# yuw444/fastF

Measured on AMD Instinct MI355X. Metric: BAM records/sec -> deduped UMI matrix; achieved HBM GB/s vs roofline, higher is better.
Workload: dtype u64

## Files before the change

fastf_amd/_lib.py:

```python
import ctypes as C
import os
import subprocess

HERE = os.path.dirname(os.path.abspath(__file__))
ROOT = os.path.dirname(HERE)
_LIB = os.environ.get("FASTF_LIB_OVERRIDE") or os.path.join(HERE, "lib", "libfastf_amd.so")
_CLI = os.path.join(HERE, "bin", "fastF")


class FastfError(RuntimeError):
    pass


def lib_path():
    return _LIB


def cli_path():
    return _CLI


def build(force=False):
    args = ["make", "-s", "-C", os.path.join(HERE, "csrc")]
    if force:
# ... 80 lines not shown
    "fastf_cap_summary_row", "fastf_cap_thresholds", "fastf_cap_realised", "fastf_dev_cell_hits", "fastf_dev_cell_decisions",
]


def _one_hip_runtime():
    import importlib.util
    import sys
    if "torch" in sys.modules or os.environ.get("FASTF_SYSTEM_HIP") == "1":
        return
    try:
        spec = importlib.util.find_spec("torch")
    except (ImportError, ValueError):
        spec = None
    if spec is None or not spec.origin:
        return
    rt = os.path.join(os.path.dirname(spec.origin), "lib", "libamdhip64.so")
    if os.path.exists(rt):
        C.CDLL(rt, mode=C.RTLD_GLOBAL)


def hip_runtimes_loaded():
    with open("/proc/self/maps") as f:
        return sorted({ln.split()[-1] for ln in f if "libamdhip64" in ln})


def lib():
    global _lib
    if _lib is not None:
        return _lib
    if not os.path.exists(_LIB):
        raise FastfError("%s is missing: run `python -c 'import __graft_entry__ as g; g.build()'` "
                         "(there is no Python/CPU fallback for the engine)" % _LIB)
    _one_hip_runtime()
    L = C.CDLL(_LIB, mode=C.RTLD_GLOBAL)
    vp, u64, u32, sz = C.c_void_p, C.c_uint64, C.c_uint32, C.c_size_t
    L.fastf_last_error.restype = C.c_char_p
    L.fastf_version.restype = C.c_char_p
    L.fastf_kernel_names.restype = C.c_char_p
    L.fastf_dev_probe_capacity.argtypes = [vp, u64, C.POINTER(u64)]
    L.fastf_engine_push_pinned.argtypes = [vp, vp]
    L.fastf_engine_wait_input.argtypes = [vp]
    L.fastf_pinned_alloc.argtypes = [sz]
    L.fastf_pinned_alloc.restype = vp
    L.fastf_pinned_free.argtypes = [vp]
    L.fastf_pinned_register.argtypes = [vp, sz]
    L.fastf_pinned_unregister.argtypes = [vp]
    L.fastf_mt_seed.argtypes = [C.POINTER(MT), u32]
    L.fastf_mt_next.argtypes = [C.POINTER(MT)]
    L.fastf_mt_next.restype = u32
    L.fastf_mt_fill.argtypes = [C.POINTER(MT), vp, sz]
    L.fastf_mt_skip.argtypes = [C.POINTER(MT), u64]
    L.fastf_draw_threshold.argtypes = [C.c_float]
    L.fastf_draw_threshold.restype = u64
    L.fastf_sample_cells.argtypes = [sz, C.c_float, C.c_uint, vp, C.POINTER(sz), C.POINTER(u64)]
    L.fastf_pack_umi.argtypes = [C.c_char_p, sz, C.POINTER(u32)]
    L.fastf_pack_umi.restype = u32
    L.fastf_keydict_create.restype = vp
    L.fastf_keydict_destroy.argtypes = [vp]
    L.fastf_keydict_add.argtypes = [vp, C.c_char_p, sz]
    L.fastf_keydict_add.restype = u64
    L.fastf_keydict_pack.argtypes = [vp, C.c_char_p, sz]
    L.fastf_keydict_pack.restype = u64
    L.fastf_keydict_pack_many.argtypes = [vp, vp, sz, sz, vp, vp]
    L.fastf_keydict_pack_many.restype = None
    L.fastf_engine_create.argtypes = [C.POINTER(EngineConfig), C.POINTER(vp)]
    L.fastf_engine_destroy.argtypes = [vp]
    L.fastf_engine_destroy.restype = None
    L.fastf_engine_push.argtypes = [vp, C.POINTER(Batch)]
    L.fastf_engine_push_draws.argtypes = [vp, C.POINTER(Batch), vp, sz]
    L.fastf_engine_finish.argtypes = [vp, C.POINTER(Coo), C.POINTER(u64 * 3)]
    L.fastf_engine_lend_rows.argtypes = [vp, vp, sz]
    L.fastf_engine_umi_rows.argtypes = [vp, C.POINTER(UmiRows)]
    L.fastf_engine_reset.argtypes = [vp]
    L.fastf_engine_device_records.argtypes = [vp, C.POINTER(u64), u32]
    L.fastf_engine_reseed.argtypes = [vp, u32, u64]
    L.fastf_engine_key_bits.argtypes = [vp, C.POINTER(u32), C.POINTER(u32), C.POINTER(u32), C.POINTER(u32)]
    L.fastf_engine_set_timing.argtypes = [vp, C.c_int]
    L.fastf_engine_get_timing.argtypes = [vp, C.c_int, C.POINTER(C.c_double), C.POINTER(u64)]
    L.fastf_dev_count_hits.argtypes = [vp, vp, u64, vp, vp]
    L.fastf_dev_count_hits_blocked.argtypes = [vp, vp, u64, vp, vp, vp]
    L.fastf_dev_block_bytes.argtypes = [vp, u64, C.POINTER(u64)]
    L.fastf_dev_block_records.argtypes = [vp, vp, vp, vp, u64, vp, vp]
    L.fastf_dev_set_regions.argtypes = [vp, vp, u32, u64, vp, vp]
    if hasattr(L, "fastf_dev_draw_bits") or not os.environ.get("FASTF_LIB_OVERRIDE"):
        L.fastf_dev_draw_bits.argtypes = [vp, vp, u64, vp, vp]
    if hasattr(L, "fastf_dev_mt_decisions"):
        L.fastf_dev_mt_decisions.argtypes = [vp, u32, u64, u64, vp, vp]
    L.fastf_dev_probe_pack.argtypes = [vp, vp, vp, vp, vp, u64, vp, u64, vp, vp, u64, vp, vp, u32, vp]
    if hasattr(L, "fastf_dev_probe_pack_wide"):
        L.fastf_dev_probe_pack_wide.argtypes = [vp, vp, vp, vp, vp, vp, u64, vp, u64, vp, vp, vp, u64, vp, vp, u32, vp]
        L.fastf_dev_adopt_wide.argtypes = [vp, vp, vp, u64, vp]
        L.fastf_engine_is_wide.argtypes = [vp]
    L.fastf_dev_sort.argtypes = [vp, vp, vp, vp, u64, u32, u32, C.POINTER(C.c_int), vp]
    L.fastf_dev_reduce.argtypes = [vp, vp, vp, u64, vp, vp, vp, vp, u32, vp]
    L.fastf_dev_rows_gather.argtypes = [vp, vp, vp, vp, vp, vp]
    L.fastf_engine_skip_bits.argtypes = [vp, C.POINTER(u32)]
    L.fastf_engine_sort_passes.argtypes = [vp, u32, C.POINTER(u32)]
    L.fastf_engine_table_modes.argtypes = [vp, C.POINTER(C.c_int), C.POINTER(C.c_int)]
    L.fastf_dev_umi_rows.argtypes = [vp, vp, vp, u64, vp, vp, vp, vp]
    L.fastf_dev_reserve.argtypes = [vp, u64, u64]
    L.fastf_dev_error_bits.argtypes = [vp, C.POINTER(u64)]
    L.fastf_dev_clear_error_bits.argtypes = [vp, u64, vp]
    L.fastf_lists_load_mem.argtypes = [C.c_char_p, sz, C.c_char_p, sz, C.c_float, C.c_uint, C.POINTER(ListsStruct)]
    L.fastf_lists_load.argtypes = [C.c_char_p, C.c_char_p, C.c_float, C.c_uint, C.POINTER(ListsStruct)]
    L.fastf_lists_free.argtypes = [C.POINTER(ListsStruct)]
    L.fastf_lists_free.restype = None
    L.fastf_bam_open.argtypes = [C.c_char_p, C.c_int]
    L.fastf_bam_open.restype = vp
    L.fastf_bam_read_batch.argtypes = [vp, vp, vp, vp, vp, vp, vp, sz]
    L.fastf_bam_read_batch.restype = C.c_long
    L.fastf_bam_close.argtypes = [vp]
    L.fastf_bam_close.restype = None
    L.fastf_bam_stats.argtypes = [vp, C.POINTER(C.c_uint64), C.POINTER(C.c_uint64), C.POINTER(C.c_uint64)]
    L.fastf_bam_stats.restype = None
    L.fastf_format_matrix.argtypes = [C.c_char_p, C.c_float, C.c_float, C.POINTER(u64 * 3), sz, sz,
                                      C.POINTER(Coo), C.POINTER(vp), C.POINTER(sz)]
    L.fastf_format_umi_rows.argtypes = [C.POINTER(UmiRows), C.POINTER(vp), C.POINTER(sz)]
    L.fastf_keydict_intern.argtypes = [vp, C.c_char_p, sz]
    L.fastf_keydict_intern.restype = u64
    L.fastf_keydict_decode.argtypes = [vp, u64, C.c_char_p, sz]
    L.fastf_keydict_decode.restype = C.c_long
    L.fastf_taghist_create.argtypes = [C.c_int, C.POINTER(vp)]
    L.fastf_taghist_destroy.argtypes = [vp]
    L.fastf_taghist_destroy.restype = None
    L.fastf_taghist_push.argtypes = [vp, vp, vp, sz]
    L.fastf_taghist_finish.argtypes = [vp, C.POINTER(TagHistResult)]
    L.fastf_crb_text.argtypes = [C.c_char_p, C.POINTER(vp), C.POINTER(sz), C.POINTER(u64)]
    L.fastf_extract_text.argtypes = [C.c_char_p, C.c_char_p, C.c_int, C.POINTER(vp), C.POINTER(sz), C.POINTER(u64), C.POINTER(u64)]
    L.fastf_freq_text.argtypes = [C.c_char_p, sz, sz, C.POINTER(vp), C.POINTER(sz), C.POINTER(u64)]
    L.fastf_filter.argtypes = [C.c_char_p, C.c_char_p, C.c_char_p, C.c_char_p, C.c_char_p, C.c_uint32, C.c_uint32, C.c_float,
                               C.c_int, C.POINTER(u64), C.POINTER(u64)]
    L.fastf_filter_draws.argtypes = [C.c_uint32, u64, u64, vp]
    L.fastf_filter_draws_host.argtypes = [C.c_uint32, u64, u64, vp]
    L.fastf_filter_rand_at.argtypes = [C.c_uint32, u64]
    L.fastf_filter_rand_at.restype = C.c_uint32
    L.fastf_filter_draw_passes.argtypes = [C.c_uint32, C.c_float]
    L.fastf_taghist_reserve_device.argtypes = [vp, sz]
    L.fastf_taghist_reserve_device.restype = vp
    L.fastf_taghist_stream.argtypes = [vp]
    L.fastf_taghist_stream.restype = vp
    L.fastf_taghist_push_device.argtypes = [vp, vp, sz]
    L.fastf_bam_read_tags.argtypes = [vp, vp, C.c_char_p, C.c_char_p, C.c_int, vp, vp, sz, C.POINTER(u64)]
    L.fastf_bam_read_tags.restype = C.c_long
    L.read_bam.argtypes = [C.c_char_p]
    L.read_bam.restype = vp
    L.print_CB_node.argtypes = [vp, vp]
    L.print_CB_node.restype = None
    L.free_CB_node.argtypes = [vp]
    L.free_CB_node.restype = None
    L.extract_bam.argtypes = [C.c_char_p, C.c_char_p, C.c_int]
    L.extract_bam.restype = None
    fp = C.POINTER(C.c_float)
    L.fastf_sweep.argtypes = [C.c_char_p, C.c_char_p, C.c_char_p, C.c_char_p, fp, u32, fp, u32, u32, u32]
    L.fastf_sweep_parse_rates.argtypes = [C.c_char_p, C.c_int, fp, u32, C.POINTER(u32)]
    L.fastf_sweep_check_grid.argtypes = [fp, u32, fp, u32]
    L.fastf_sweep_point_dir.argtypes = [C.c_float, C.c_float, C.c_char_p, sz]
    L.fastf_sweep_header.restype = C.c_char_p
    L.fastf_sweep_cells_from_coo.argtypes = [C.POINTER(Coo), u32, vp, vp, C.POINTER(u64)]
    L.fastf_sweep_summary_row.argtypes = [C.c_float, C.c_float, u32, C.POINTER(u64 * 3), u64, u64, vp, vp, u32, C.c_char_p, sz]
    L.fastf_dev_mt_decisions_multi.argtypes = [vp, u32, u64, u64, vp, u32, vp, u64, vp]
    L.fastf_dev_cell_summary.argtypes = [vp, vp, vp, vp, u32, vp, vp, vp]
    L.fastf_cap.argtypes = [C.c_char_p, C.c_char_p, C.c_char_p, C.c_char_p, fp, u32, vp, u32, u32, u32]
    L.fastf_cap_parse_caps.argtypes = [C.c_char_p, vp, u32, C.POINTER(u32)]
    L.fastf_cap_check_grid.argtypes = [fp, u32, vp, u32]
    L.fastf_cap_point_dir.argtypes = [C.c_float, u64, C.c_char_p, sz]
    L.fastf_cap_header.restype = C.c_char_p
# ... 15 lines not shown
```

fastf_amd/csrc/umi_engine.hip:

```cpp
#include "umi_kernels.hpp"
#include "sweep_kernels.hpp"
#include "cap_kernels.hpp"

#include <algorithm>
#include <cstdarg>
#include <cstdio>
#include <cstdlib>
#include <cstring>
#include <mutex>
#include <new>
#include <stdexcept>
#include <chrono>
#include <string>
#include <thread>
#include <vector>

extern "C" {
#include "fastf_amd.h"
#include "host_io.h"
#include "mt_jump.h"
}

using namespace fastf;

// ... 123 lines not shown
static int copy_h2d_on(void* d_dst, const void* h_src, size_t bytes, hipStream_t s) {
    std::lock_guard<std::mutex> lk(g_bounce.mu);
    if (g_bounce.ready()) return 1;
    for (size_t o = 0; o < bytes; o += HostBounce::BYTES) {
        const size_t n = std::min(bytes - o, HostBounce::BYTES);
        memcpy(g_bounce.p, (const char*)h_src + o, n);
        HIP_OK(hipMemcpyAsync((char*)d_dst + o, g_bounce.p, n, hipMemcpyHostToDevice, s));
        HIP_OK(hipStreamSynchronize(s));
    }
    return 0;
}

struct KernelTimer {
    std::vector<std::pair<hipEvent_t, hipEvent_t>> ev;
    size_t used = 0;
};

struct fastf_multi;
struct fastf_engine {
    fastf_multi* multi = nullptr;
    int device = 0;
    hipStream_t s_compute = nullptr, s_copy = nullptr, s_mt = nullptr;
    hipEvent_t ev_mt = nullptr;
    KeyLayout L{};
    u32 cell_bits = 0, feat_bits = 0, n_cells = 0, n_features = 0;
    u64 threshold = 0;
    u32 n_shards = 1, shard_rank = 0;
    DevBuf tab_cells, tab_feats;
    Table cells{}, feats{};
    DevBuf img_cells, img_genes;
    DevBuf d_cell_filter; MissFilter cell_filter{nullptr, 0};
    CellLds lds_cells{}; GeneLds lds_genes{};
    bool cell16 = false;
    bool use_lds_cells = false, use_lds_genes = false; u32 genes_blocks_per_cu = 1, cells_blocks_per_cu = 1;
    fastf_mt_t mt{};
    u32 mt_seed0 = 0; u64 mt_skip0 = 0;
    u64 mt_hits = 0;
    u64 mt_abs0 = 0;
    bool mt_live = false;
    DevBuf d_ring; u64 ring_len = 0;
    u32 ring_carry = 0;
    DevBuf d_dbits;
    DevBuf d_mtwords;
    bool mtwords_kept = false; u32 mtwords_seed = 0; u64 mtwords_skip = 0, mtwords_n = 0;
    bool cap_lds_attr = false;
    DevBuf d_mt; bool mt_on_device = false;
    u32 mt_dev_idx = MT_N;
    DevBuf d_mtsub, d_mtpoly, d_mtseat, d_mtseq;
    u64 draws_up = 0;
    u64 draws_valid = 0;
    u64 batch_cap = 0;
    struct Slot {
        void* h_stage = nullptr;
        void* h_draws = nullptr;
        DevBuf d_stage;
        hipEvent_t ev_copy = nullptr, ev_done = nullptr;
        u64* h_small = nullptr;
        bool busy = false; u64 n = 0; bool external = false;
    } slot[2];
    int cur = 0;
    const u32* cur_umi_ext = nullptr;
    u64 inflight_records = 0;
    u64 key_cap = 0;
    DevBuf d_keys, d_tmp;
    DevBuf d_small;
    u64* h_small = nullptr;
    DevBuf d_feature, d_cell, d_count, d_ukeys, d_ncopy;
    u32* h_coo = nullptr; u64 h_coo_cap = 0, h_nnz = 0;
    bool h_coo_pinned = false; u32 h_coo_uses = 0;
    u32* lent_rows = nullptr; u64 lent_cap = 0;
    u32* rows_at = nullptr; u64 rows_stride = 0;
    std::vector<u32> h_ufeature, h_ucell, h_uumi, h_ncopy;
    std::vector<uint8_t> h_unonnull;
    u64 total_records = 0, hits_so_far = 0, keys_so_far = 0;
    u64 c_sampled = 0, c_valid = 0;
    bool finished = false; int sorted_in_tmp = 0; u64 n_sorted = 0;
    u32 skip_bits = 0;
    bool fully_sorted = false;
    DevBuf d_cellidx, d_tilecnt, d_tilebase, d_binbase, d_cnt;
    DevBuf d_halfhits;
    DevBuf d_segkeys;
    DevBuf d_segcount, d_segprefix, d_tileseg;
    u32 giant_parity = 0;
    u32 seg_n = 0; u64 seg_stride = 0;
    DevBuf d_rgn_phys, d_rgn_hist, d_rgn_blk;
    u32 rgn_hist_n = 0, rgn_hist_shift = 0;
    bool stream_mode = false, store_regions = false;
    bool narrow = false, genes_one_family = false;
    u64 slots_used = 0, slot_cap = 0; u32 rgn_n = 0, rgn_cap = 0;
    DevBuf d_scanblk;
    DevBuf d_rg_feature, d_rg_cell, d_rg_count, d_rg_ukeys, d_spanrows, d_spanbase, d_giant;
    u32 rg_n = 0; bool rg_umi = false;
    bool wide = false, long_umi = false; u32 group_bits = 0;
    u32 sub_bits = 0, row_split = 0;
    bool finish_queued = false;
    DevBuf d_vals, d_vtmp;
    bool timing = false;
    hipEvent_t t_ev[2] = {nullptr, nullptr};
    double t_scatter_ms = 0; u64 t_scatter_n = 0;
    double t_k1_ms = 0; u64 t_k1_n = 0;
    double t_k1b_ms = 0; u64 t_k1b_n = 0;
    double t_k3_ms = 0; u64 t_k3_n = 0;
    double t_count_ms = 0; u64 t_count_n = 0;
    double t_gather_ms = 0; u64 t_gather_n = 0;
};

enum { SM_KEYCOUNT = 0, SM_COUNTERS = 32, SM_NNZ = 64, SM_NROWS_U = 65, SM_N = 66, SM_RUNNING = 96, SM_DRAWBASE = 128, SM_WORDS = 160 };

static int set_scatter_lds_limit();
static u32 g_cu_count = 256;
static int multi_create(const fastf_engine_config_t* cfg, fastf_engine* e);
static void multi_destroy(fastf_engine* e);
static int multi_push(fastf_engine* e, const fastf_batch_t* b, bool pinned);
static int multi_finish(fastf_engine* e, fastf_coo_t* coo, uint64_t counters[3]);
static int multi_umi_rows(fastf_engine* e, fastf_umi_rows_t* rows);
static int multi_reset(fastf_engine* e, bool reseed, u32 seed, u64 skip);
static int multi_device_records(const fastf_engine* e, uint64_t* records, u32 n);
static size_t scatter_smem_bytes(u32 ipt = SORT_IPT) {
    return (size_t)ipt * SORT_THREADS * 8 + (size_t)SORT_WAVES * RADIX * 4 + RADIX * 4 * 2 + 64;
}

static u32 h_slot_hash(u64 key) {
    const u32 h = (u32)key * 0x9E3779B1u + (u32)(key >> 32) * 0x85EBCA77u;
    return h ^ (h >> 15);
}

static int build_table(const u64* keys, u32 n, DevBuf& buf, Table& t, const char* what) {
    u32 cap = 64;
    while (cap < 2ull * n) cap <<= 1;
    std::vector<uint4> slots(cap, make_uint4(0, 0, 0, 0));
    for (u32 i = 0; i < n; ++i) {
        const u64 k = keys[i];
        if (k == 0) return set_err("%s key %u is 0 (unpackable string?)", what, i);
        u32 h = h_slot_hash(k) & (cap - 1);
        for (;;) {
            uint4& s = slots[h];
            const u64 sk = ((u64)s.y << 32) | s.x;
            if (sk == 0) { s.x = (u32)k; s.y = (u32)(k >> 32); s.z = i + 1; break; }
            if (sk == k) return set_err("duplicate %s key at index %u (first occurrence wins in the reference; dedup before create)", what, i);
            h = (h + 1) & (cap - 1);
        }
    }
    if (buf.ensure((size_t)cap * sizeof(uint4))) return 1;
    if (copy_h2d(buf.p, slots.data(), (size_t)cap * sizeof(uint4))) return 1;
    t.slots = (const uint4*)buf.p;
    t.mask = cap - 1;
    return 0;
}

static u32 h_filter_bit(u64 key) {
    const u32 h = (u32)key * 0x85EBCA77u + (u32)(key >> 32) * 0xC2B2AE3Du;
    return h ^ (h >> 13);
}

static int build_cell_filter(fastf_engine* e, const u64* keys, u32 n) {
    if (n == 0 || getenv("FASTF_NO_CELL_FILTER")) return 0;
    u32 bits = 1u << 15;
    while (bits < 10ull * n && bits < (1u << 18)) bits <<= 1;
    std::vector<u32> w(bits / 32, 0u);
    for (u32 i = 0; i < n; ++i) { const u32 b = h_filter_bit(keys[i]) & (bits - 1); w[b >> 5] |= 1u << (b & 31); }
    if (e->d_cell_filter.ensure(bits / 8)) return 1;
    if (copy_h2d(e->d_cell_filter.p, w.data(), bits / 8)) return 1;
    e->cell_filter.bits = (const u32*)e->d_cell_filter.p; e->cell_filter.mask = bits - 1;
    if (hipFuncSetAttribute(reinterpret_cast<const void*>(probe_cells_filtered_kernel), hipFuncAttributeMaxDynamicSharedMemorySize,
                            (int)(bits / 8)) != hipSuccess) { e->cell_filter.bits = nullptr; }
    return 0;
}

// ... 209 lines not shown
        const u32 passes = (kb - fs + 7) / 8;
        e->skip_bits = sk ? (u32)atoi(sk) : (kb > 8 * passes ? kb - 8 * passes : 0);
        if (e->skip_bits >= fs) e->skip_bits = 0;
        if (e->wide) e->skip_bits = 0;
    }
    e->n_shards = cfg->n_shards; e->shard_rank = cfg->shard_rank;
    e->mt_seed0 = cfg->mt_seed; e->mt_skip0 = cfg->mt_skip;

    int rc = 0;
    do {
        int prio_lo = 0, prio_hi = 0;
        const char* sp = getenv("FASTF_STREAM_PRIORITY");
        const bool high = sp && sp[0] == '1' && hipDeviceGetStreamPriorityRange(&prio_lo, &prio_hi) == hipSuccess && prio_hi != prio_lo;
        auto mk = [&](hipStream_t* s) { return high ? hipStreamCreateWithPriority(s, hipStreamNonBlocking, prio_hi) : hipStreamCreateWithFlags(s, hipStreamNonBlocking); };
        if (mk(&e->s_compute) != hipSuccess ||
            mk(&e->s_copy) != hipSuccess ||
            mk(&e->s_mt) != hipSuccess ||
            hipEventCreateWithFlags(&e->ev_mt, hipEventDisableTiming) != hipSuccess ||
            hipEventCreateWithFlags(&e->slot[0].ev_copy, hipEventDisableTiming) != hipSuccess ||
            hipEventCreateWithFlags(&e->slot[1].ev_copy, hipEventDisableTiming) != hipSuccess ||
            hipEventCreateWithFlags(&e->slot[0].ev_done, hipEventDisableTiming) != hipSuccess ||
            hipEventCreateWithFlags(&e->slot[1].ev_done, hipEventDisableTiming) != hipSuccess ||
            hipEventCreate(&e->t_ev[0]) != hipSuccess || hipEventCreate(&e->t_ev[1]) != hipSuccess) {
            rc = set_err("stream/event creation failed"); break;
        }
        lap("streams and events");
        if ((rc = build_table((const u64*)cfg->cell_keys, cfg->n_cells, e->tab_cells, e->cells, "cell"))) break;
        if ((rc = build_table((const u64*)cfg->feature_keys, cfg->n_features, e->tab_feats, e->feats, "feature"))) break;
        {
            const char* lt = getenv("FASTF_LDS_TABLES");
            if (!(lt && lt[0] == '0')) {
                const char* lc = getenv("FASTF_LDS_CELLS");
                if (!(lc && lc[0] == '0') && (rc = build_cell_lds(e, (const u64*)cfg->cell_keys, cfg->n_cells))) break;
                if (!e->use_lds_cells && (rc = build_cell_filter(e, (const u64*)cfg->cell_keys, cfg->n_cells))) break;
                if ((rc = build_gene_lds(e, (const u64*)cfg->feature_keys, cfg->n_features))) break;
            }
        }
        lap("tables built and uploaded");
        if ((rc = e->d_small.ensure(SM_WORDS * sizeof(u64)))) break;
        if (hipHostMalloc((void**)&e->h_small, SM_WORDS * sizeof(u64), hipHostMallocDefault) != hipSuccess) {
            rc = set_err("hipHostMalloc failed"); break;
        }
        if (hipMemset(e->d_small.p, 0, SM_WORDS * sizeof(u64)) != hipSuccess) { rc = set_err("memset failed"); break; }
        lap("counters allocated and cleared");
        if (set_scatter_lds_limit()) {
            rc = set_err("cannot raise dynamic LDS limit to %zu bytes", scatter_smem_bytes()); break;
        }
        lap("kernel attributes (code object loaded)");
        e->batch_cap = cfg->batch_records ? cfg->batch_records : (4ull << 20);
        e->key_cap = cfg->key_capacity;
        e->stream_mode = e->use_lds_genes && !e->wide && e->n_shards == 1 && !getenv("FASTF_NO_STREAM_K1B") && !getenv("FASTF_PUSH_TILE_FORM");
        {
            const char* bw = getenv("FASTF_BLOCK_WIDE");
            e->narrow = e->stream_mode && e->genes_one_family && e->lds_genes.vmin + e->lds_genes.range <= 0xFFFFFFFFull &&
                        e->L.umi_bits <= 24 && !(bw && bw[0] == '1');
        }
    } while (0);
    if (rc) { fastf_engine_destroy(e); return 1; }
    *out = e;
    return 0;
} FASTF_CATCH_INT

extern "C" void fastf_engine_destroy(fastf_engine_t* e) FASTF_TRY {
    if (!e) return;
    if (e->multi) { multi_destroy(e); delete e; return; }
    (void)hipSetDevice(e->device);
    (void)hipDeviceSynchronize();
    for (int i = 0; i < 2; ++i) {
        fastf_engine::Slot& sl = e->slot[i];
        if (sl.h_stage) (void)hipHostFree(sl.h_stage);
        if (sl.h_draws) (void)hipHostFree(sl.h_draws);
        if (sl.h_small) (void)hipHostFree(sl.h_small);
        sl.d_stage.release();
        if (sl.ev_copy) (void)hipEventDestroy(sl.ev_copy);
        if (sl.ev_done) (void)hipEventDestroy(sl.ev_done);
        if (e->t_ev[i]) (void)hipEventDestroy(e->t_ev[i]);
    }
    if (e->h_small) (void)hipHostFree(e->h_small);
    if (e->h_coo) { if (e->h_coo_pinned) pin_unreg(e->h_coo); fastf_big_free(e->h_coo, (size_t)e->h_coo_cap * 12); }
    e->d_ring.release(); e->d_mt.release(); e->d_dbits.release(); e->d_mtwords.release(); e->d_mtsub.release(); e->d_mtpoly.release(); e->d_mtseat.release(); e->d_mtseq.release();
    DevBuf* all[] = {&e->tab_cells, &e->tab_feats, &e->img_cells, &e->img_genes, &e->d_cell_filter, &e->d_keys, &e->d_tmp, &e->d_small, &e->d_feature, &e->d_cell,
                     &e->d_count, &e->d_ukeys, &e->d_ncopy, &e->d_cellidx, &e->d_tilecnt, &e->d_tilebase, &e->d_binbase, &e->d_cnt, &e->d_rg_feature, &e->d_rg_cell, &e->d_rg_count, &e->d_rg_ukeys, &e->d_spanrows, &e->d_spanbase, &e->d_giant, &e->d_scanblk,
                     &e->d_halfhits, &e->d_segcount, &e->d_segprefix, &e->d_tileseg, &e->d_segkeys, &e->d_vals, &e->d_vtmp,
                     &e->d_rgn_phys, &e->d_rgn_hist, &e->d_rgn_blk};
    for (DevBuf* b : all) b->release();
    if (e->s_compute) (void)hipStreamDestroy(e->s_compute);
    if (e->s_copy) (void)hipStreamDestroy(e->s_copy);
    if (e->s_mt) (void)hipStreamDestroy(e->s_mt);
    if (e->ev_mt) (void)hipEventDestroy(e->ev_mt);
    delete e;
} FASTF_CATCH_VOID

extern "C" int fastf_engine_table_modes(const fastf_engine_t* e, int* cells_in_lds, int* genes_in_lds) FASTF_TRY {
    if (!e) return set_err("null engine");
    if (cells_in_lds) *cells_in_lds = e->use_lds_cells;
    if (genes_in_lds) *genes_in_lds = e->use_lds_genes ? (e->lds_genes.direct ? 2 : 1) : 0;
    return 0;
} FASTF_CATCH_INT

extern "C" int fastf_engine_cell_scratch_bytes(const fastf_engine_t* e, uint32_t* bytes) FASTF_TRY {
    if (!e || !bytes) return set_err("null argument");
    *bytes = (e->multi ? e->n_cells <= 65535u : e->cell16) ? 2u : 4u;
    return 0;
} FASTF_CATCH_INT

extern "C" int fastf_engine_sort_passes(const fastf_engine_t* e, uint32_t flags, uint32_t* passes) FASTF_TRY {
    if (!e || !passes) return set_err("null argument");
    *passes = sort_passes(e->L.total_bits, (flags & FASTF_SORT_SKIP_LOW) ? e->skip_bits : 0);
    return 0;
} FASTF_CATCH_INT

extern "C" int fastf_engine_skip_bits(const fastf_engine_t* e, uint32_t* bits) FASTF_TRY {
    if (!e || !bits) return set_err("null argument");
    *bits = e->skip_bits;
    return 0;
} FASTF_CATCH_INT

extern "C" int fastf_engine_key_bits(const fastf_engine_t* e, uint32_t* cell_bits, uint32_t* feature_bits,
                                     uint32_t* umi_bits, uint32_t* total_bits) FASTF_TRY {
    if (!e) return set_err("null engine");
    if (cell_bits) *cell_bits = e->cell_bits;
    if (feature_bits) *feature_bits = e->feat_bits;
    if (umi_bits) *umi_bits = 1 + e->L.umi_bits + e->L.len_bits;
    if (total_bits) *total_bits = e->L.total_bits;
    return 0;
} FASTF_CATCH_INT

static u64 max_tiles_for(u64 n, u64 tile) { return (n + tile - 1) / tile + 1; }

static u32 choose_sort_ipt(u64 n) {
    const char* f = getenv("FASTF_SORT_IPT");
    if (f) { int v = atoi(f); if (v >= 1 && v <= SORT_IPT) return (u32)v; }
    const u64 max_ipt = std::min<u64>(7, SORT_IPT), slots = 4ull * g_cu_count;
    const u64 per_round_max = slots * SORT_THREADS * max_ipt;
    const u64 rounds = std::max<u64>(1, (n + per_round_max - 1) / per_round_max);
    const u64 per_thread = (n + rounds * slots * SORT_THREADS - 1) / (rounds * slots * SORT_THREADS);
    return (u32)std::min<u64>(max_ipt, std::max<u64>(1, per_thread));
}

static int reserve_workspace(fastf_engine* e, u64 max_records, u64 max_keys, u64 tile_records = 0) {
    const u64 t1 = max_tiles_for(std::max(max_records, tile_records), K1_TILE);
    const u64 ts = max_tiles_for(max_keys, (u64)choose_sort_ipt(max_keys) * SORT_THREADS);
    if (max_records && e->d_cellidx.ensure(max_records * sizeof(u32))) return 1;
    if (e->d_tilecnt.bytes < t1 * sizeof(u32)) {
        if (e->d_tilecnt.ensure(t1 * sizeof(u32))) return 1;
        HIP_OK(hipDeviceSynchronize());
        HIP_OK(hipMemset(e->d_tilecnt.p, 0, e->d_tilecnt.bytes));
    }
    if (e->d_tilebase.ensure(t1 * sizeof(u64))) return 1;
    if (e->d_halfhits.ensure(t1 * 16 * sizeof(u32))) return 1;
    if (e->d_tileseg.ensure((ts + 8) * sizeof(TileSeg))) return 1;
    if (e->d_binbase.ensure(RADIX * sizeof(u32))) return 1;
    if (e->d_cnt.ensure((ts + 4) * RADIX * sizeof(u32))) return 1;
    return 0;
}

extern "C" int fastf_dev_reserve(fastf_engine_t* e, uint64_t max_records, uint64_t max_keys) FASTF_TRY {
    if (!e) return set_err("null engine");
    if (e->multi) return set_err("fastf_dev_reserve: device-level calls take a single-device engine");
    HIP_OK(hipSetDevice(e->device));
    return reserve_workspace(e, max_records, max_keys);
} FASTF_CATCH_INT

static bool dbg_sync_on() { static int v = -1; if (v < 0) v = getenv("FASTF_DEBUG_SYNC") != nullptr; return v != 0; }
static void dbg_sync(hipStream_t s, const char* what) {
    if (!dbg_sync_on()) return;
    const hipError_t e1 = hipStreamSynchronize(s), e2 = hipGetLastError();
    fprintf(stderr, "[sync] %s: %s %s\n", what, hipGetErrorString(e1), e2 == hipSuccess ? "" : hipGetErrorString(e2));
    fflush(stderr);
}

static void t_begin(fastf_engine* e, hipStream_t s) { if (e->timing) (void)hipEventRecord(e->t_ev[0], s); }
static void t_end(fastf_engine* e, hipStream_t s, double* acc, u64* cnt) {
    if (!e->timing) return;
    (void)hipEventRecord(e->t_ev[1], s);
    (void)hipEventSynchronize(e->t_ev[1]);
    float ms = 0;
    if (hipEventElapsedTime(&ms, e->t_ev[0], e->t_ev[1]) == hipSuccess) { *acc += ms; *cnt += 1; }
}

extern "C" int fastf_engine_set_timing(fastf_engine_t* e, int on) FASTF_TRY {
    if (!e) return set_err("null engine");
    if (e->multi) return set_err("fastf_engine_set_timing: device-level calls take a single-device engine");
    e->timing = on != 0;
    e->t_scatter_ms = e->t_k1_ms = e->t_k1b_ms = e->t_k3_ms = e->t_count_ms = e->t_gather_ms = 0;
    e->t_scatter_n = e->t_k1_n = e->t_k1b_n = e->t_k3_n = e->t_count_n = e->t_gather_n = 0;
    return 0;
} FASTF_CATCH_INT
extern "C" int fastf_engine_get_timing(fastf_engine_t* e, int which, double* total_ms, uint64_t* launches) FASTF_TRY {
    if (!e) return set_err("null engine");
    const double ms[6] = {e->t_k1_ms, e->t_scatter_ms, e->t_k3_ms, e->t_count_ms, e->t_k1b_ms, e->t_gather_ms};
    const u64 n[6] = {e->t_k1_n, e->t_scatter_n, e->t_k3_n, e->t_count_n, e->t_k1b_n, e->t_gather_n};
    if (which < 0 || which > 5) return set_err("bad timer index");
    *total_ms = ms[which]; *launches = n[which];
    return 0;
} FASTF_CATCH_INT

static u64* g_k1_stamps = nullptr;
extern "C" void fastf_debug_set_k1_stamps(void* p) { g_k1_stamps = (u64*)p; }

static void launch_scan_tiles(fastf_engine* e, int slot, hipStream_t s, u32* in, u64* out, u32 T, u64* total_out, u64* running, u64* base_out) {
    constexpr u32 CHUNK = 16u * 1024u;
    const u32 n_blk = (T + CHUNK - 1) / CHUNK;
    if (n_blk <= 1 || n_blk > 64 || e->d_scanblk.ensure(2 * 64 * sizeof(u64))) {
        hipLaunchKernelGGL(scan_tiles_kernel<16>, dim3(1), dim3(1024), 0, s, in, out, T, total_out, running, base_out, (u64*)nullptr);
        return;
    }
    u64* const blk = (u64*)e->d_scanblk.p + 64 * slot;
    hipLaunchKernelGGL(scan_tiles_kernel<16>, dim3(n_blk), dim3(1024), 0, s, in, out, T, (u64*)nullptr, (u64*)nullptr, (u64*)nullptr, blk);
    hipLaunchKernelGGL(scan_fix_kernel<16>, dim3(n_blk), dim3(1024), 0, s, out, T, (const u64*)blk, n_blk, total_out, running, base_out);
}

static int launch_probe_cells(fastf_engine* e, const u64* cb, u64 n, u64* d_total_out, hipStream_t s,
                              u64* d_running = nullptr, u64* d_base_out = nullptr, void* blk = nullptr) {
    if (reserve_workspace(e, blk ? 0 : n, 0, n)) return 1;
    const u32 tiles = (u32)((n + K1_TILE - 1) / K1_TILE);
    const CellOut cout = blk ? CellOut{blk, blk_run_bytes(e->cell16, e->narrow), blk_cell_off(e->narrow)} : CellOut{e->d_cellidx.p, 0u, 0u};
    t_begin(e, s);
    if (e->use_lds_cells) {
        const u32 grid = std::min<u32>(e->cells_blocks_per_cu * g_cu_count, (tiles + 1) / 2);
        if (e->cells_blocks_per_cu >= 2)
            hipLaunchKernelGGL(probe_cells_lds_kernel<true>, dim3(grid), dim3(1024), e->lds_cells.bytes, s, cb, n, e->lds_cells,
                               cout, e->cell16, (u32*)e->d_tilecnt.p, (u32*)e->d_halfhits.p, tiles);
        else
            hipLaunchKernelGGL(probe_cells_lds_kernel<false>, dim3(grid), dim3(1024), e->lds_cells.bytes, s, cb, n, e->lds_cells,
                               cout, e->cell16, (u32*)e->d_tilecnt.p, (u32*)e->d_halfhits.p, tiles);
    } else if (e->cell_filter.bits) {
        const u32 grid = std::min<u32>(tiles, 4 * g_cu_count);
        hipLaunchKernelGGL(probe_cells_filtered_kernel, dim3(grid), dim3(K1_THREADS), (e->cell_filter.mask + 1u) / 8u, s, cb, n,
                           e->cells, e->cell_filter, cout, e->cell16, (u32*)e->d_tilecnt.p, (u32*)e->d_halfhits.p, tiles);
    } else {
        hipLaunchKernelGGL(probe_cells_kernel<0>, dim3(tiles), dim3(K1_THREADS), 0, s, cb, n, e->cells,
                           cout, e->cell16, (u32*)e->d_tilecnt.p, (u32*)e->d_halfhits.p);
    }
    t_end(e, s, &e->t_k1_ms, &e->t_k1_n);
    dbg_sync(s, "K1a probe_cells");
    launch_scan_tiles(e, 0, s, (u32*)e->d_tilecnt.p, (u64*)e->d_tilebase.p, tiles, d_total_out, d_running, d_base_out);
    dbg_sync(s, "K1a tile scan");
    HIP_OK(hipGetLastError());
    return 0;
}

extern "C" int fastf_dev_count_hits(fastf_engine_t* e, const uint64_t* d_cb_key, uint64_t n,
                                    uint64_t* d_hits_out, void* stream) FASTF_TRY {
    if (!e) return set_err("null engine");
    if (e->multi) return set_err("fastf_dev_count_hits: device-level calls take a single-device engine");
    HIP_OK(hipSetDevice(e->device));
    hipStream_t s = (hipStream_t)stream;
    if (n == 0) { HIP_OK(hipMemsetAsync(d_hits_out, 0, sizeof(u64), s)); return 0; }
    return launch_probe_cells(e, (const u64*)d_cb_key, n, (u64*)d_hits_out, s);
} FASTF_CATCH_INT

static bool stream_k1b_possible(const fastf_engine* e) {
    return e->use_lds_genes && e->n_shards <= (u32)MAX_SHARDS && !getenv("FASTF_NO_STREAM_K1B");
}

extern "C" int fastf_dev_block_bytes(const fastf_engine_t* e, uint64_t n, uint64_t* bytes) FASTF_TRY {
    if (!e || !bytes) return set_err("null argument");
    *bytes = 0;
    if (e->multi || e->wide || !stream_k1b_possible(e)) return 0;
    *bytes = ((n + BLK_RECS - 1) / BLK_RECS) * (u64)blk_run_bytes(e->cell16, e->narrow);
    return 0;
} FASTF_CATCH_INT

static void launch_block_records(const fastf_engine* e, const u64* gx, const u32* umi, const u32* meta, u64 n, void* blk, hipStream_t s) {
    const u64 units = (n + BLK_RECS - 1) / BLK_RECS;
    const dim3 grid((u32)std::min<u64>((units + 3) / 4, 16ull * g_cu_count));
    if (e->narrow) hipLaunchKernelGGL(block_records_kernel<true>, grid, dim3(256), 0, s, gx, umi, meta, n, (unsigned char*)blk,
                                      blk_run_bytes(e->cell16, true), e->lds_genes.family, e->L);
    else hipLaunchKernelGGL(block_records_kernel<false>, grid, dim3(256), 0, s, gx, umi, meta, n, (unsigned char*)blk,
                            blk_run_bytes(e->cell16, false), 0u, e->L);
}

extern "C" int fastf_dev_block_records(fastf_engine_t* e, const uint64_t* d_gx_key, const uint32_t* d_umi, const uint32_t* d_meta,
                                       uint64_t n, void* d_blocked, void* stream) FASTF_TRY {
    if (!e || !d_blocked) return set_err("null argument");
    if (e->multi) return set_err("fastf_dev_block_records: device-level calls take a single-device engine");
    HIP_OK(hipSetDevice(e->device));
    if (n == 0) return 0;
    launch_block_records(e, (const u64*)d_gx_key, d_umi, d_meta, n, d_blocked, (hipStream_t)stream);
    HIP_OK(hipGetLastError());
    dbg_sync((hipStream_t)stream, "block_records");
    return 0;
} FASTF_CATCH_INT

extern "C" int fastf_dev_count_hits_blocked(fastf_engine_t* e, const uint64_t* d_cb_key, uint64_t n, void* d_blocked,
                                            uint64_t* d_hits_out, void* stream) FASTF_TRY {
    if (!e || !d_blocked) return set_err("null argument");
    if (e->multi) return set_err("fastf_dev_count_hits_blocked: device-level calls take a single-device engine");
    HIP_OK(hipSetDevice(e->device));
    hipStream_t s = (hipStream_t)stream;
    if (n == 0) { HIP_OK(hipMemsetAsync(d_hits_out, 0, sizeof(u64), s)); return 0; }
    return launch_probe_cells(e, (const u64*)d_cb_key, n, (u64*)d_hits_out, s, nullptr, nullptr, d_blocked);
} FASTF_CATCH_INT

static int launch_draw_bits(u64 threshold, const u32* d_draws, u64 n, u32* d_bits, hipStream_t s, u64 first = 0, u64 ring_mask = ~0ull) {
    if (n == 0) return 0;
    const u32 grid = (u32)std::min<u64>((n + 255) / 256 + 1, 8ull * g_cu_count);
    hipLaunchKernelGGL(draw_bits_kernel, dim3(grid), dim3(256), 0, s, d_draws, n, threshold, d_bits, first, ring_mask);
    HIP_OK(hipGetLastError());
    return 0;
}
struct PlaneOut { const u64* thresholds; u32 n; u64* planes; u64 stride; };
static int launch_draw_planes(const PlaneOut& po, const u32* d_draws, u64 n, hipStream_t s) {
    if (n == 0) return 0;
    const u32 grid = (u32)std::min<u64>((n + 255) / 256 + 1, 8ull * g_cu_count);
    for (u32 j0 = 0; j0 < po.n; j0 += PLANES_MAX) {
        PlaneSet ps{}; ps.n = std::min<u32>(PLANES_MAX, po.n - j0);
        for (u32 j = 0; j < ps.n; ++j) ps.threshold[j] = po.thresholds[j0 + j];
        hipLaunchKernelGGL(draw_planes_kernel, dim3(grid), dim3(256), 0, s, d_draws, n, ps, po.planes + (u64)j0 * po.stride, po.stride);
    }
    HIP_OK(hipGetLastError());
    return 0;
}
static int launch_mt_decisions(hipStream_t s, u32* d_mt, DevBuf& words, u32* d_ring, u64 first, u64 count, u64 ring_mask, u64 threshold, const PlaneOut* po = nullptr,
                               bool words_only = false) {
    if (count == 0) return 0;
    if (words.bytes < count * 4) {
        if (words.p) HIP_OK(hipStreamSynchronize(s));
        if (words.ensure(std::max<u64>(count * 4, 1u << 20))) return 1;
// ... 160 lines not shown
extern "C" int fastf_dev_cell_decisions(fastf_engine_t* e, uint64_t n, const void* d_blocked, uint32_t seed, uint64_t skip, uint64_t n_draws,
                                        const uint64_t* d_thresholds, uint32_t* d_bits_out, void* stream) FASTF_TRY {
    if (!e || (n_draws && (!d_bits_out || !d_thresholds))) return set_err("null argument");
    if (e->multi) return set_err("fastf_dev_cell_decisions: device-level calls take a single-device engine");
    if ((uintptr_t)d_bits_out & 7) return set_err("fastf_dev_cell_decisions: the plane is 8-byte aligned");
    HIP_OK(hipSetDevice(e->device));
    hipStream_t s = (hipStream_t)stream;
    auto sync = [&]() -> int {
        if (hipStreamSynchronize(s) != hipSuccess) return set_err("the generator or decision kernels failed: %s", hipGetErrorString(hipGetLastError()));
        return 0;
    };
    if (!n_draws) return sync();
    HIP_OK(hipMemsetAsync(d_bits_out, 0, (size_t)((n_draws + 63) / 64) * 8, s));
    if (n == 0 || !e->n_cells) return sync();
    if (!d_blocked && e->d_cellidx.bytes < n * (e->cell16 ? 2u : 4u)) return set_err("fastf_dev_cell_decisions: no cell scratch for %llu records: fastf_dev_count_hits comes first", (unsigned long long)n);
    const u64 tiles = (n + K1_TILE - 1) / K1_TILE;
    if (e->d_tilebase.bytes < tiles * sizeof(u64) || e->d_halfhits.bytes < tiles * 16 * sizeof(u32)) return set_err("fastf_dev_cell_decisions: no hit counts for %llu records: fastf_dev_count_hits comes first", (unsigned long long)n);
    if (!(e->mtwords_kept && e->mtwords_seed == seed && e->mtwords_skip == skip && e->mtwords_n >= n_draws)) {
        fastf_mt_t mt; fastf_mt_seed(&mt, seed); fastf_mt_skip(&mt, skip);
        if (e->d_mtseat.ensure(sizeof mt)) return 1;
        if (copy_h2d_on(e->d_mtseat.p, &mt, sizeof mt, s)) return 1;
        u32 idx = (u32)mt.idx;
        if (launch_mt_decisions_par(e, s, (u32*)e->d_mtseat.p, &idx, e->d_mtwords, nullptr, 0, n_draws, ~0ull, 0, nullptr, true)) return 1;
        e->mtwords_kept = true; e->mtwords_seed = seed; e->mtwords_skip = skip; e->mtwords_n = n_draws;
    }
    const u64 units = (n + BLK_RECS - 1) / BLK_RECS;
    const u32 grid = (u32)std::min<u64>((units + 3) / 4, 8ull * g_cu_count);
    hipLaunchKernelGGL(cell_decisions_kernel, dim3(grid), dim3(256), 0, s, cell_scratch_of(e, d_blocked), e->cell16, n, (const u64*)e->d_tilebase.p,
                       (const u32*)e->d_halfhits.p, (const u32*)e->d_mtwords.p, n_draws, (const u64*)d_thresholds, e->n_cells, (u64*)d_bits_out);
    HIP_OK(hipGetLastError());
    return sync();
} FASTF_CATCH_INT

extern "C" void* fastf_devmem_alloc(int device, size_t bytes) FASTF_TRY {
    void* p = nullptr;
    if (hipSetDevice(device) != hipSuccess || hipMalloc(&p, bytes ? bytes : 1) != hipSuccess) {
        set_err("device allocation of %zu bytes failed: %s", bytes, hipGetErrorString(hipGetLastError()));
        return nullptr;
    }
    return p;
} FASTF_CATCH_(return nullptr)
extern "C" void fastf_devmem_free(void* p) { if (p) (void)hipFree(p); }
extern "C" int fastf_devmem_copy(void* dst, const void* src, size_t bytes) FASTF_TRY {
    if (!bytes) return 0;
    HIP_OK(hipMemcpy(dst, src, bytes, hipMemcpyDefault));
    return 0;
} FASTF_CATCH_INT
extern "C" int fastf_devmem_zero(void* dst, size_t bytes) FASTF_TRY {
    if (!bytes) return 0;
    HIP_OK(hipMemset(dst, 0, bytes));
    return 0;
} FASTF_CATCH_INT
extern "C" int fastf_devmem_sync(void) FASTF_TRY {
    HIP_OK(hipDeviceSynchronize());
    return 0;
} FASTF_CATCH_INT

extern "C" int fastf_dev_draw_bits(fastf_engine_t* e, const uint32_t* d_draws, uint64_t n_draws, uint32_t* d_bits_out, void* stream) FASTF_TRY {
    if (!e || (n_draws && (!d_draws || !d_bits_out))) return set_err("null argument");
    if (e->multi) return set_err("fastf_dev_draw_bits: device-level calls take a single-device engine");
    HIP_OK(hipSetDevice(e->device));
    return launch_draw_bits(e->threshold, d_draws, n_draws, d_bits_out, (hipStream_t)stream);
} FASTF_CATCH_INT

#define NO_WIDE(e, what) do { if ((e)->wide) return set_err(what ": this engine's keys are wider than 64 bits — this call moves one 64 bits word per key (fastf_dev_probe_pack_wide / fastf_dev_adopt_wide + fastf_engine_finish and the host-buffer API take wide keys)"); } while (0)

static void stream_geometry(const fastf_engine* e, u64 tiles, u32* grid, u64* region) {
    const u32 waves = (e->genes_blocks_per_cu >= 2 ? K1S_THREADS : K1S_THREADS_ROOMY) / WAVE;
    const u64 units = std::max<u64>(tiles, 1) * (K1_TILE / K1S_UNIT);
    const u64 g = std::max<u64>(1, std::min<u64>((units + 4 * waves - 1) / (4 * waves), (u64)std::min<u32>(e->genes_blocks_per_cu, 2) * g_cu_count));
    const u64 rounds = (units + g * waves - 1) / (g * waves);
    *grid = (u32)g; *region = ((rounds + K1S_SUB - 1) / K1S_SUB) * waves * K1S_UNIT;
}
struct RegionAppend { u64 slot0; u32 rgn0; };

static int grow_regions(fastf_engine* e, u32 need);
static int launch_probe(fastf_engine* e, const u64* cb, const u64* gx, const u32* umi, const u32* meta, u64 n,
                        const u32* dbits, u64 n_draws, const u64* draw_base, u64* keys, u64 stride, u64* key_counts,
                        u64* counters, bool reuse_hits, hipStream_t s, u64 draw_mask = ~0ull, u64* d_running = nullptr,
                        bool segmented = false, void* blk = nullptr, const RegionAppend* app = nullptr,
                        u64* wide_vals = nullptr, const u32* wide_ext = nullptr) {
    if (segmented && !app) { e->seg_n = 0; e->rgn_hist_n = 0; }
    if (n == 0) return 0;
    if (!reuse_hits && launch_probe_cells(e, cb, n, nullptr, s, d_running, d_running ? const_cast<u64*>(draw_base) : nullptr, blk)) return 1;
    const u32 tiles = (u32)((n + K1_TILE - 1) / K1_TILE);
    PackParams p{};
    p.cell = e->d_cellidx.p; p.cell16 = e->cell16; p.gx = gx; p.umi = umi; p.meta = meta; p.n = n;
    p.tile_base = (const u64*)e->d_tilebase.p;
    p.dbits = dbits && n_draws ? dbits : (const u32*)e->d_small.p; p.n_draws = dbits ? n_draws : 0; p.draw_base = draw_base; p.draw_mask = draw_mask;
    p.feats = e->feats;
    p.L = e->L;
    p.n_shards = e->n_shards;
    p.keys = keys; p.shard_stride = stride; p.key_counts = key_counts; p.counters = counters;
    p.stamps = g_k1_stamps;
    p.n_tiles = tiles;
    p.genes = e->lds_genes;
    p.blk = (const unsigned char*)blk;
    if (e->wide) {
        if (segmented || blk) return set_err("internal error: wide keys take the tile form");
        if (!wide_vals && (e->n_shards != 1 || keys != (u64*)e->d_keys.p)) return set_err("internal error: wide keys go through the engine's own key store");
        p.vals = wide_vals ? wide_vals : (u64*)e->d_vals.p; p.wide_feat_bits = e->feat_bits; p.wide_sub_bits = e->sub_bits;
        p.umi_ext = wide_vals ? wide_ext : e->cur_umi_ext;
    }
    const bool no_stream = getenv("FASTF_NO_STREAM_K1B") != nullptr;
    const bool stream_shards = !segmented && !e->wide && e->n_shards > 1 && e->n_shards <= (u32)MAX_SHARDS && e->use_lds_genes && !no_stream;
    if (blk && !(segmented || stream_shards)) return set_err("FASTF_PROBE_BLOCKED needs the streaming K1b (fastf_dev_block_bytes returns 0 otherwise)");
    t_begin(e, s);
    if (segmented || stream_shards) {
        u32 grid; u64 region;
        stream_geometry(e, tiles, &grid, &region);
        const u32 n_rgn = grid * (u32)K1S_SUB, rgn0 = app ? app->rgn0 : 0u;
        if (stream_shards) {
            if (e->d_segkeys.ensure((size_t)n_rgn * region * sizeof(u64))) return 1;
            p.keys = (u64*)e->d_segkeys.p;
        } else if ((u64)n_rgn * region > stride) return set_err("segmented key output needs %llu slots, the buffer has %llu (fastf_dev_probe_capacity)",
                                                                (unsigned long long)((u64)n_rgn * region), (unsigned long long)stride);
        if (app) {
            if (e->rgn_cap < rgn0 + n_rgn) return set_err("internal error: region tables too small");
        } else {
            if (e->rgn_n) return set_err("device-level K1 on an engine that holds pushed chunks: fastf_engine_reset first");
            if (grow_regions(e, n_rgn)) return 1;
        }
        if (e->d_segprefix.ensure(((size_t)n_rgn + 1) * sizeof(u64))) return 1;
        StreamParams sp{(const u32*)e->d_halfhits.p, region, (u64*)e->d_segcount.p + rgn0,
                        stream_shards ? nullptr : (u32*)e->d_rgn_hist.p + (size_t)rgn0 * RADIX, (u64*)e->d_rgn_phys.p + rgn0,
                        app ? app->slot0 : 0ull, e->skip_bits};
        const int variant = (e->genes_blocks_per_cu >= 2 ? 0 : 4) | (e->cell16 ? 2 : 0) | (e->lds_genes.direct ? 1 : 0);
#define FPS(R, C, D) do { if (blk && e->narrow) hipLaunchKernelGGL((filter_pack_stream_kernel<R, C, D, true, true>), dim3(grid), dim3(R ? K1S_THREADS_ROOMY : K1S_THREADS), e->lds_genes.bytes, s, p, sp); \
                          else if (blk) hipLaunchKernelGGL((filter_pack_stream_kernel<R, C, D, true>), dim3(grid), dim3(R ? K1S_THREADS_ROOMY : K1S_THREADS), e->lds_genes.bytes, s, p, sp); \
                          else hipLaunchKernelGGL((filter_pack_stream_kernel<R, C, D, false>), dim3(grid), dim3(R ? K1S_THREADS_ROOMY : K1S_THREADS), e->lds_genes.bytes, s, p, sp); } while (0)
        switch (variant) {
        case 0: FPS(false, false, false); break; case 1: FPS(false, false, true); break;
        case 2: FPS(false, true, false); break;  case 3: FPS(false, true, true); break;
        case 4: FPS(true, false, false); break;  case 5: FPS(true, false, true); break;
        case 6: FPS(true, true, false); break;   default: FPS(true, true, true); break;
        }
#undef FPS
        if (stream_shards) {
            hipLaunchKernelGGL(shard_partition_kernel, dim3(n_rgn), dim3(SP_THREADS), 0, s, (const u64*)e->d_segkeys.p, (const u64*)e->d_segcount.p,
                               region, e->L.cell_shift, e->n_shards, keys, stride, key_counts, counters + 3);
        } else if (app) {
            hipLaunchKernelGGL(seg_scan_kernel, dim3(1), dim3(1024), 0, s, (const u64*)e->d_segcount.p + rgn0, n_rgn, (u64*)e->d_segprefix.p, key_counts, true);
        } else {
            hipLaunchKernelGGL(seg_scan_kernel, dim3(1), dim3(1024), 0, s, (const u64*)e->d_segcount.p, n_rgn, (u64*)e->d_segprefix.p, key_counts, false);
            e->seg_n = n_rgn; e->seg_stride = region;
            e->rgn_hist_n = n_rgn; e->rgn_hist_shift = e->skip_bits;
        }
    } else if (e->use_lds_genes) {
        const u32 grid = std::min<u32>(tiles, e->genes_blocks_per_cu * g_cu_count);
        if (e->genes_blocks_per_cu >= 2) hipLaunchKernelGGL((filter_pack_kernel<true, false>), dim3(grid), dim3(K1B_THREADS), e->lds_genes.bytes, s, p);
        else hipLaunchKernelGGL((filter_pack_kernel<true, true>), dim3(grid), dim3(K1B_THREADS), e->lds_genes.bytes, s, p);
    } else {
        hipLaunchKernelGGL(filter_pack_kernel<false>, dim3(tiles), dim3(K1B_THREADS), 0, s, p);
    }
    HIP_OK(hipGetLastError());
    t_end(e, s, &e->t_k1b_ms, &e->t_k1b_n);
    dbg_sync(s, blk ? "K1b filter_pack (blocked)" : "K1b filter_pack");
    return 0;
}

extern "C" int fastf_dev_probe_pack(fastf_engine_t* e, const uint64_t* d_cb_key, const uint64_t* d_gx_key,
                                    const uint32_t* d_umi, const uint32_t* d_meta, uint64_t n,
                                    const uint32_t* d_draws, uint64_t n_draws, const uint64_t* d_draw_base,
                                    uint64_t* d_keys_out, uint64_t shard_stride, uint64_t* d_key_counts,
                                    uint64_t* d_counters, uint32_t flags, void* stream) FASTF_TRY {
    if (!e) return set_err("null engine");
    if (e->multi) return set_err("fastf_dev_probe_pack: device-level calls take a single-device engine");
    HIP_OK(hipSetDevice(e->device));
    NO_WIDE(e, "fastf_dev_probe_pack");
    const bool seg = (flags & FASTF_PROBE_SEGMENTED) != 0, blocked = (flags & FASTF_PROBE_BLOCKED) != 0;
    if (seg && !(e->n_shards == 1 && e->use_lds_genes))
        return set_err("FASTF_PROBE_SEGMENTED needs a single shard and the gene table in LDS (fastf_dev_probe_capacity returns 0 otherwise)");
    if (blocked && !d_gx_key) return set_err("FASTF_PROBE_BLOCKED: d_gx_key must point at the blocked buffer");
    if (n && n_draws && !d_draws) return set_err("null d_draws");
    if (!(flags & FASTF_PROBE_DRAW_BITS) && n && n_draws) {
        if (e->d_dbits.ensure(((n_draws + 63) / 64) * 8)) return 1;
        if (launch_draw_bits(e->threshold, d_draws, n_draws, (u32*)e->d_dbits.p, (hipStream_t)stream)) return 1;
        d_draws = (const uint32_t*)e->d_dbits.p;
    }
    return launch_probe(e, (const u64*)d_cb_key, blocked ? nullptr : (const u64*)d_gx_key, d_umi, d_meta, n, d_draws, n_draws,
                        (const u64*)d_draw_base, (u64*)d_keys_out, shard_stride, (u64*)d_key_counts, (u64*)d_counters,
                        (flags & FASTF_PROBE_REUSE_HITS) != 0, (hipStream_t)stream, ~0ull, nullptr, seg,
                        blocked ? const_cast<uint64_t*>(d_gx_key) : nullptr);
} FASTF_CATCH_INT

extern "C" int fastf_engine_is_wide(const fastf_engine_t* e) { return e && !e->multi && e->wide ? 1 : 0; }

extern "C" int fastf_dev_probe_pack_wide(fastf_engine_t* e, const uint64_t* d_cb_key, const uint64_t* d_gx_key, const uint32_t* d_umi,
                                         const uint32_t* d_meta, const uint32_t* d_umi_ext, uint64_t n,
                                         const uint32_t* d_draws, uint64_t n_draws, const uint64_t* d_draw_base,
                                         uint64_t* d_keys_out, uint64_t* d_vals_out, uint64_t shard_stride, uint64_t* d_key_counts,
                                         uint64_t* d_counters, uint32_t flags, void* stream) FASTF_TRY {
    if (!e) return set_err("null engine");
    if (e->multi) return set_err("fastf_dev_probe_pack_wide: device-level calls take a single-device engine");
    if (!e->wide) return set_err("fastf_dev_probe_pack_wide: this engine's keys fit 64 bits (fastf_dev_probe_pack)");
    if (flags & (FASTF_PROBE_SEGMENTED | FASTF_PROBE_BLOCKED)) return set_err("fastf_dev_probe_pack_wide: wide keys take the tile form (no SEGMENTED / BLOCKED)");
    if (!d_keys_out || !d_vals_out) return set_err("null key or value output");
    if (e->long_umi && !d_umi_ext && n) return set_err("this engine was created with umi_max_bases > 16: d_umi_ext (bases 17.. of every UMI, zeros where none) is needed");
    HIP_OK(hipSetDevice(e->device));
    if (n && n_draws && !d_draws) return set_err("null d_draws");
    if (!(flags & FASTF_PROBE_DRAW_BITS) && n && n_draws) {
        if (e->d_dbits.ensure(((n_draws + 63) / 64) * 8)) return 1;
        if (launch_draw_bits(e->threshold, d_draws, n_draws, (u32*)e->d_dbits.p, (hipStream_t)stream)) return 1;
        d_draws = (const uint32_t*)e->d_dbits.p;
    }
    return launch_probe(e, (const u64*)d_cb_key, (const u64*)d_gx_key, d_umi, d_meta, n, d_draws, n_draws, (const u64*)d_draw_base,
                        (u64*)d_keys_out, shard_stride, (u64*)d_key_counts, (u64*)d_counters, (flags & FASTF_PROBE_REUSE_HITS) != 0,
                        (hipStream_t)stream, ~0ull, nullptr, false, nullptr, nullptr, (u64*)d_vals_out, d_umi_ext);
} FASTF_CATCH_INT

extern "C" int fastf_dev_probe_capacity(const fastf_engine_t* e, uint64_t n, uint64_t* key_slots) FASTF_TRY {
    if (!e || !key_slots) return set_err("null argument");
    *key_slots = 0;
    if (e->wide) return 0;
    if (!(e->n_shards == 1 && e->use_lds_genes) || getenv("FASTF_NO_STREAM_K1B")) return 0;
    u32 grid; u64 region;
    stream_geometry(e, (n + K1_TILE - 1) / K1_TILE, &grid, &region);
    *key_slots = (u64)grid * K1S_SUB * region;
    return 0;
} FASTF_CATCH_INT

static u64* g_stamps = nullptr;
extern "C" void fastf_debug_set_stamps(void* p) { g_stamps = (u64*)p; }
static u32 tile_grid(u32 T) {
    static int cap = -1;
    if (cap < 0) { const char* c = getenv("FASTF_TILE_GRID_CAP"); cap = c ? atoi(c) : 32 * (int)g_cu_count; if (cap < 8) cap = 8; }
    return std::min<u32>((T + 7u) & ~7u, (u32)cap & ~7u);
}
static size_t scatter_smem_bytes_vals(u32 ipt) { return scatter_smem_bytes(ipt) + (size_t)ipt * SORT_THREADS * 8; }
static void launch_scatter(u32 shift, u32 T, hipStream_t s, const u64* src, u64* dst, const u64* d_n, const u32* cnt,
                           const u32* bin_tot, u32 ipt, const SegMap seg = SegMap{nullptr, nullptr, 0, 0},
                           const u64* vsrc = nullptr, u64* vdst = nullptr) {
    T = tile_grid(T);
    if (vsrc) {
        hipLaunchKernelGGL((scatter_kernel<-1, false, true>), dim3(T), dim3(SORT_THREADS), scatter_smem_bytes_vals(ipt), s, src, dst, d_n, cnt, bin_tot, ipt, shift,
                           SegMap{nullptr, nullptr, 0, 0}, (u64*)nullptr, vsrc, vdst);
        return;
    }
#define SC(SH) hipLaunchKernelGGL(scatter_kernel<SH>, dim3(T), dim3(SORT_THREADS), scatter_smem_bytes(ipt), s, src, dst, d_n, cnt, bin_tot, ipt, shift, seg, g_stamps)
    if (seg.prefix) {
        hipLaunchKernelGGL((scatter_kernel<-1, true>), dim3(T), dim3(SORT_THREADS), scatter_smem_bytes(ipt), s, src, dst, d_n, cnt, bin_tot, ipt, shift, seg, g_stamps);
        return;
    }
    const bool rt = (shift & 7u) != 0 || getenv("FASTF_SORT_RUNTIME_SHIFT");
    switch (rt ? 64u : shift) {
    case 0: SC(0); break;  case 8: SC(8); break;  case 16: SC(16); break; case 24: SC(24); break;
    case 32: SC(32); break; case 40: SC(40); break; case 48: SC(48); break; case 56: SC(56); break;
    default: SC(-1); break;
    }
#undef SC
}

static int set_scatter_lds_limit() {
    const void* fns[10] = {(const void*)scatter_kernel<0>, (const void*)scatter_kernel<8>, (const void*)scatter_kernel<16>,
                           (const void*)scatter_kernel<24>, (const void*)scatter_kernel<32>, (const void*)scatter_kernel<40>,
                           (const void*)scatter_kernel<48>, (const void*)scatter_kernel<56>, (const void*)scatter_kernel<-1>,
                           (const void*)scatter_kernel<-1, true>};
    for (const void* f : fns)
        if (hipFuncSetAttribute(f, hipFuncAttributeMaxDynamicSharedMemorySize, (int)scatter_smem_bytes()) != hipSuccess) return 1;
    if (hipFuncSetAttribute((const void*)scatter_kernel<-1, false, true>, hipFuncAttributeMaxDynamicSharedMemorySize, (int)scatter_smem_bytes_vals(SORT_IPT)) != hipSuccess) return 1;
    if (hipFuncSetAttribute((const void*)scatter_regions_kernel, hipFuncAttributeMaxDynamicSharedMemorySize, (int)scatter_smem_bytes()) != hipSuccess) return 1;
    return 0;
}

static int launch_sort(fastf_engine* e, u64* keys, u64* tmp, const u64* d_n, u64 max_n, u32 key_bits, u32 low_bit,
                       int* sorted_in_tmp, hipStream_t s, bool segmented_input = false, u64* vals = nullptr, u64* vtmp = nullptr) {
    if (key_bits > 64) return set_err("key_bits %u > 64", key_bits);
    const u32 passes = sort_passes(key_bits, low_bit);
    *sorted_in_tmp = (int)(passes & 1);
    if (max_n == 0) return 0;
    if (max_n >= (1ull << 32)) return set_err("sort of %llu keys: limit is 2^32-1 per shard", (unsigned long long)max_n);
    if (reserve_workspace(e, 0, max_n)) return 1;
    const u32 ipt = choose_sort_ipt(max_n);
    const u32 T = (u32)((max_n + (u64)ipt * SORT_THREADS - 1) / ((u64)ipt * SORT_THREADS));
    u32* bintot = (u32*)e->d_binbase.p; u32* cnt = (u32*)e->d_cnt.p;
    SegMap seg{nullptr, nullptr, 0, 0};
    bool walk = false;
    if (segmented_input) {
        if (!e->seg_n) return set_err("FASTF_SORT_SEGMENTED without a preceding FASTF_PROBE_SEGMENTED probe_pack");
        if (passes == 0) return set_err("segmented keys need at least one sort pass");
        static const bool no_walk = getenv("FASTF_NO_REGION_WALK") != nullptr;
        walk = e->rgn_hist_n == e->seg_n && e->rgn_hist_shift == low_bit && !no_walk && !vals;
        if (!walk) {
            if (!e->seg_stride) return set_err("internal error: regions without a common stride need their histograms");
            seg = SegMap{(const u64*)e->d_segprefix.p, (const TileSeg*)e->d_tileseg.p, e->seg_n, e->seg_stride};
            hipLaunchKernelGGL(seg_tiles_kernel, dim3(std::min<u32>((T + 255) / 256, 1024)), dim3(256), 0, s, seg.prefix, seg.n_seg,
                               seg.stride, ipt * SORT_THREADS, (TileSeg*)e->d_tileseg.p);
        }
    }
    const SegMap none{nullptr, nullptr, 0, 0};
    for (u32 q = 0; q < passes; ++q) {
        const u64* src = (q & 1) ? tmp : keys;
        u64* dst = (q & 1) ? keys : tmp;
        const u32 shift = low_bit + 8 * q;
        if (q == 0 && walk) {
            const u32 R = e->seg_n, n_blk = (R + RGN_BLK - 1) / RGN_BLK;
            if (e->d_rgn_blk.ensure((size_t)n_blk * RADIX * sizeof(u32))) return 1;
            hipLaunchKernelGGL(rgn_scan_blocks_kernel, dim3(n_blk), dim3(RADIX), 0, s, (u32*)e->d_rgn_hist.p, R, (u32*)e->d_rgn_blk.p);
            hipLaunchKernelGGL(rgn_scan_fix_kernel, dim3(n_blk), dim3(RADIX), 0, s, (u32*)e->d_rgn_hist.p, R, (const u32*)e->d_rgn_blk.p, n_blk, bintot);
            t_begin(e, s);
            hipLaunchKernelGGL(scatter_regions_kernel, dim3(tile_grid(R)), dim3(SORT_THREADS), scatter_smem_bytes(ipt), s, src, dst,
                               (const u64*)e->d_rgn_phys.p, (const u64*)e->d_segcount.p, (const u32*)e->d_rgn_hist.p, (const u32*)bintot, R, ipt, shift,
                               max_n >= (24ull << 20));
            t_end(e, s, &e->t_scatter_ms, &e->t_scatter_n);
            e->rgn_hist_n = 0;
            dbg_sync(s, "K2 sort pass (region walk)");
            continue;
        }
        t_begin(e, s);
        if (q == 0 && seg.prefix) hipLaunchKernelGGL(tile_count_kernel<true>, dim3(tile_grid(T)), dim3(SORT_THREADS), 0, s, src, d_n, shift, cnt, ipt, seg);
        else hipLaunchKernelGGL(tile_count_kernel<false>, dim3(tile_grid(T)), dim3(SORT_THREADS), 0, s, src, d_n, shift, cnt, ipt, none);
        t_end(e, s, &e->t_count_ms, &e->t_count_n);
        hipLaunchKernelGGL(row_scan_kernel, dim3(RADIX), dim3(1024), 0, s, cnt, d_n, bintot, ipt);
        t_begin(e, s);
        if (vals) launch_scatter(shift, T, s, src, dst, d_n, (const u32*)cnt, (const u32*)bintot, ipt, none, (q & 1) ? vtmp : vals, (q & 1) ? vals : vtmp);
        else launch_scatter(shift, T, s, src, dst, d_n, (const u32*)cnt, (const u32*)bintot, ipt, q == 0 ? seg : none);
        t_end(e, s, &e->t_scatter_ms, &e->t_scatter_n);
        dbg_sync(s, "K2 sort pass");
    }
    HIP_OK(hipGetLastError());
    return 0;
}

extern "C" int fastf_dev_set_regions(fastf_engine_t* e, const uint64_t* d_counts, uint32_t n_regions, uint64_t stride,
                                     uint64_t* d_n_out, void* stream) FASTF_TRY {
    if (!e || !d_counts || !d_n_out) return set_err("null argument");
    if (e->multi) return set_err("fastf_dev_set_regions: device-level calls take a single-device engine");
    if (n_regions == 0 || stride == 0) return set_err("fastf_dev_set_regions: no regions");
    HIP_OK(hipSetDevice(e->device));
    if (e->d_segprefix.ensure(((size_t)n_regions + 1) * sizeof(u64))) return 1;
    hipLaunchKernelGGL(seg_scan_kernel, dim3(1), dim3(1024), 0, (hipStream_t)stream, (const u64*)d_counts, (u32)n_regions, (u64*)e->d_segprefix.p, (u64*)d_n_out);
    HIP_OK(hipGetLastError());
    e->seg_n = n_regions; e->seg_stride = stride; e->rgn_hist_n = 0;
    return 0;
} FASTF_CATCH_INT

extern "C" int fastf_dev_sort(fastf_engine_t* e, uint64_t* d_keys, uint64_t* d_tmp, const uint64_t* d_n,
                              uint64_t max_n, uint32_t key_bits, uint32_t flags, int* sorted_in_tmp, void* stream) FASTF_TRY {
    if (!e) return set_err("null engine");
    if (e->multi) return set_err("fastf_dev_sort: device-level calls take a single-device engine");
    NO_WIDE(e, "fastf_dev_sort");
    HIP_OK(hipSetDevice(e->device));
    int dummy = 0;
    return launch_sort(e, (u64*)d_keys, (u64*)d_tmp, (const u64*)d_n, max_n, key_bits,
                       (flags & FASTF_SORT_SKIP_LOW) ? e->skip_bits : 0,
                       sorted_in_tmp ? sorted_in_tmp : &dummy, (hipStream_t)stream, (flags & FASTF_SORT_SEGMENTED) != 0);
} FASTF_CATCH_INT

static u32 k3_grid(u64 max_n, int dedup) {
    static int per_cu[3] = {-1, -1, -1};
    if (per_cu[dedup] < 0) {
        const char* c = getenv("FASTF_K3_PER_CU");
        per_cu[dedup] = c ? atoi(c) : 4;
        if (per_cu[dedup] < 1) per_cu[dedup] = 1;
    }
    const u64 tiles = (max_n + K3_TILE - 1) / K3_TILE;
    return (u32)std::min<u64>(std::max<u64>(tiles, 1), std::min<u64>((u64)per_cu[dedup] * g_cu_count, 4096));
}

template <bool UMI_ROWS>
static int launch_reduce_regions(fastf_engine* e, const u64* sorted, const u64* d_n, u64 max_n, u64* nrows, u32 low_skip, hipStream_t s,
                                 const u64* wide_vals = nullptr) {
    e->rg_n = 0;
    if (max_n == 0) { HIP_OK(hipMemsetAsync(nrows, 0, sizeof(u64), s)); return 0; }
    if (wide_vals && UMI_ROWS) return set_err("internal error: -u rows of wide keys");
    const int dedup = wide_vals ? 2 : (UMI_ROWS || low_skip == 0) ? 0 : 2;
    u32 G = k3_grid(max_n, dedup);
    if (dedup == 2) G = std::min<u32>(G, (wide_vals ? 2u : 3u) * g_cu_count);
    if (e->d_rg_count.ensure(max_n * 4)) return 1;
    if (UMI_ROWS ? e->d_rg_ukeys.ensure(max_n * 8) : (e->d_rg_feature.ensure(max_n * 4) || e->d_rg_cell.ensure(max_n * 4))) return 1;
    if (e->d_spanrows.ensure(4096 * sizeof(u32)) || e->d_spanbase.ensure(4097 * sizeof(u64))) return 1;
    if (dedup == 2 && !e->d_giant.p) {
        if (e->d_giant.ensure((size_t)GIANT_LIST_CAP * GIANT_ITEM_WORDS * sizeof(u64) + 64)) return 1;
        HIP_OK(hipMemsetAsync(e->d_giant.p, 0, e->d_giant.bytes, s));
    }
    u32* const giant_cnt = dedup == 2 ? (u32*)((char*)e->d_giant.p + (size_t)GIANT_LIST_CAP * GIANT_ITEM_WORDS * sizeof(u64)) : nullptr;
    const u32 parity = dedup == 2 ? (e->giant_parity ^= 1u) : 0u;
    u32* const giant_n = giant_cnt ? giant_cnt + parity : nullptr;
    ReduceParams p{};
    p.keys = sorted; p.n_ptr = d_n; p.L = e->L; p.feat_mask = (u32)((1ull << (wide_vals ? e->row_split : e->feat_bits)) - 1);
    p.err = (u64*)e->d_small.p + SM_COUNTERS + 3;
    p.feature = (u32*)e->d_rg_feature.p; p.cell = (u32*)e->d_rg_cell.p; p.count = (u32*)e->d_rg_count.p; p.ukeys = (u64*)e->d_rg_ukeys.p;
    p.span_rows = (u32*)e->d_spanrows.p;
    p.giant_list = (u64*)e->d_giant.p; p.giant_n = giant_n;
    p.giant_max = wide_vals ? (1u << 22) : GIANT_MAX;
    p.vals = wide_vals; p.wide_feat_bits = e->row_split;
    t_begin(e, s);
    if (UMI_ROWS) hipLaunchKernelGGL((reduce_windows_kernel<true>), dim3(G), dim3(K3_THREADS), 0, s, p);
    else if (dedup == 0) hipLaunchKernelGGL((reduce_windows_kernel<false>), dim3(G), dim3(K3_THREADS), 0, s, p);
    else if (wide_vals) hipLaunchKernelGGL((reduce_hashed_kernel<true, true>), dim3(G), dim3(K3H_THREADS), 0, s, p);
    else if (e->L.feat_shift > 27) hipLaunchKernelGGL((reduce_hashed_kernel<true>), dim3(G), dim3(K3H_THREADS), 0, s, p);
    else hipLaunchKernelGGL((reduce_hashed_kernel<false>), dim3(G), dim3(K3H_THREADS), 0, s, p);
    if (dedup == 2)
        hipLaunchKernelGGL(giant_groups_kernel, dim3(g_cu_count + 1), dim3(512), 0, s, wide_vals ? wide_vals : sorted, (const u64*)e->d_giant.p, giant_cnt, parity, e->L,
                           (u32*)e->d_rg_count.p, (u64*)e->d_small.p + SM_COUNTERS + 3, (const u32*)e->d_spanrows.p, G, (u64*)e->d_spanbase.p, nrows);
    else
        hipLaunchKernelGGL(span_scan_kernel, dim3(1), dim3(1024), 0, s, (const u32*)e->d_spanrows.p, G, (u64*)e->d_spanbase.p, nrows);
    HIP_OK(hipGetLastError());
    if (!UMI_ROWS) t_end(e, s, &e->t_k3_ms, &e->t_k3_n);
    dbg_sync(s, "K3 reduce + span scan + giant groups");
    e->rg_n = G; e->rg_umi = UMI_ROWS;
    return 0;
}

template <bool UMI_ROWS>
static int launch_rows_gather(fastf_engine* e, const u64* d_n, u32* feature, u32* cell, u32* count, u64* ukeys, hipStream_t s) {
    if (!e->rg_n) return 0;
    if (e->rg_umi != UMI_ROWS) return set_err("rows gather: the last reduce on this engine was of the other kind");
    t_begin(e, s);
    hipLaunchKernelGGL(rows_gather_kernel<UMI_ROWS>, dim3(e->rg_n), dim3(256), 0, s, (const u32*)e->d_rg_feature.p, (const u32*)e->d_rg_cell.p,
                       (const u32*)e->d_rg_count.p, (const u64*)e->d_rg_ukeys.p, (const u32*)e->d_spanrows.p, (const u64*)e->d_spanbase.p,
                       d_n, e->rg_n, feature, cell, count, ukeys);
    HIP_OK(hipGetLastError());
    if (!UMI_ROWS) t_end(e, s, &e->t_gather_ms, &e->t_gather_n);
    return 0;
}
// ... 826 lines not shown
```

fastf_amd/csrc/umi_kernels.hpp:

```cpp
#pragma once
#if !defined(FASTF_EXPERIMENT)
#  if defined(FASTF_X_ANY)
#    error "FASTF_X_* knobs need -DFASTF_EXPERIMENT (experiment builds only: tools/build_variant.sh)"
#  endif
#endif
#ifndef FASTF_K1_IPT
#define FASTF_K1_IPT 8
#endif
#ifndef FASTF_K1_THREADS
#define FASTF_K1_THREADS 512
#endif
#include <hip/hip_runtime.h>
#include <stdint.h>
#include <type_traits>

namespace fastf {

typedef unsigned long long u64;
typedef unsigned int u32;

constexpr int WAVE = 64;

constexpr u64 ERR_DRAWS_SHORT  = 2;
constexpr u64 ERR_UMI_TOOLONG  = 4;
// ... 298 lines not shown
    return ((u64)cell << L.cell_shift) | ((u64)feat << L.feat_shift) | (low & (0ull - (u64)nn));
}
__device__ __forceinline__ bool umi_overflows_flat(const KeyLayout L, u32 umi, u32 meta) {
    const u32 tail = L.umi_bits < 32 ? (1u << (32 - L.umi_bits)) - 1u : 0u;
    const u32 len = (meta & META_LEN_MASK) >> META_LEN_SHIFT;
    return ((meta & META_UMI_TOOLONG) != 0) | (((meta & META_UMI_NONNULL) != 0) & ((len > L.umi_max_bytes) | ((umi & tail) != 0)));
}
__device__ __forceinline__ bool umi_overflows_narrow(const KeyLayout L, u32 um) {
    const u32 len = (um & META_LEN_MASK) >> META_LEN_SHIFT;
    return ((um & META_UMI_TOOLONG) != 0) | (((um & META_UMI_NONNULL) != 0) & (len > L.umi_max_bytes));
}

__device__ __forceinline__ u64 make_val64(const KeyLayout L, u64 umi, u32 meta) {
    if (!(meta & META_UMI_NONNULL)) return 0;
    const u32 len = (meta & META_LEN_MASK) >> META_LEN_SHIFT;
    return (1ULL << (L.umi_bits + L.len_bits)) | ((umi >> (64 - L.umi_bits)) << L.len_bits) | len;
}
constexpr u32 WIDE_SUB_BITS = 17, WIDE_SUB_VAL_BITS = 51, WIDE_SUB_LEN_BITS = 4;
__device__ __forceinline__ u64 make_val_sub(u64 umi, u32 meta) {
    if (!(meta & META_UMI_NONNULL)) return 0;
    const u32 len = (meta & META_LEN_MASK) >> META_LEN_SHIFT;
    return (1ULL << WIDE_SUB_VAL_BITS) | (((umi << WIDE_SUB_LEN_BITS) | len) & ((1ULL << WIDE_SUB_VAL_BITS) - 1));
}
__device__ __forceinline__ u32 wide_sub_of(u32 umi_first_word, u32 meta) {
    static_assert(WIDE_SUB_VAL_BITS - WIDE_SUB_LEN_BITS + WIDE_SUB_BITS == 64, "the sub-group and the value's bases make up the 64 bits of bases");
    return (meta & META_UMI_NONNULL) ? umi_first_word >> (32 - WIDE_SUB_BITS) : 0u;
}
__device__ __forceinline__ bool umi_overflows_sub(u32 meta) {
    return (meta & META_UMI_TOOLONG) || ((meta & META_UMI_NONNULL) && ((meta & META_LEN_MASK) >> META_LEN_SHIFT) > 8u);
}
__device__ __forceinline__ bool umi_overflows64(const KeyLayout L, u64 umi, u32 meta) {
    if (meta & META_UMI_TOOLONG) return true;
    if (!(meta & META_UMI_NONNULL)) return false;
    const u32 len = (meta & META_LEN_MASK) >> META_LEN_SHIFT;
    return len > L.umi_max_bytes || (L.umi_bits < 64 && (umi << L.umi_bits) != 0);
}

__device__ __forceinline__ bool umi_overflows(const KeyLayout L, u32 umi, u32 meta) {
    if (meta & META_UMI_TOOLONG) return true;
    if (!(meta & META_UMI_NONNULL)) return false;
    const u32 len = (meta & META_LEN_MASK) >> META_LEN_SHIFT;
    return len > L.umi_max_bytes || (L.umi_bits < 32 && (umi << L.umi_bits) != 0);
}

__device__ __forceinline__ u32 table_probe_from(const Table t, u64 key, u32 h) {
    for (u32 i = 0; i <= t.mask; ++i) {
        const uint4 s = t.slots[h];
        const u64 k = ((u64)s.y << 32) | s.x;
        if (k == key) return s.z;
        if (k == 0) return 0;
        h = (h + 1) & t.mask;
    }
    return 0;
}

typedef __attribute__((__vector_size__(4 * sizeof(int)))) int i32x4_t;

template <int N, int AUX = 0>
__device__ __forceinline__ void table_probe_batch(const Table t, const u64 (&key)[N], u32 (&val)[N]) {
    u32 h[N]; uint4 s[N];
    const auto rsrc = __builtin_amdgcn_make_buffer_rsrc((void*)t.slots, 0, (t.mask + 1u) * 16u, 0x00020000);
#pragma unroll
    for (int j = 0; j < N; ++j) h[j] = key[j] ? (slot_hash(key[j]) & t.mask) : 0u;
#pragma unroll
    for (int j = 0; j < N; ++j) {
        const i32x4_t v = __builtin_amdgcn_raw_buffer_load_b128(rsrc, (int)(h[j] * 16u), 0, AUX);
        s[j] = make_uint4((u32)v[0], (u32)v[1], (u32)v[2], (u32)v[3]);
    }
#pragma unroll
    for (int j = 0; j < N; ++j) {
        const u64 k = ((u64)s[j].y << 32) | s[j].x;
        u32 v = 0;
        if (key[j] != 0) {
            if (k == key[j]) v = s[j].z;
            else if (k != 0) v = table_probe_from(t, key[j], (h[j] + 1) & t.mask);
        }
        val[j] = v;
    }
}

template <u32 PER>
__global__ __launch_bounds__(1024) void scan_tiles_kernel(u32* __restrict__ in, u64* __restrict__ out, u32 T,
                                                          u64* __restrict__ total_out, u64* __restrict__ running = nullptr,
                                                          u64* __restrict__ base_out = nullptr, u64* __restrict__ blk_tot = nullptr) {
    __shared__ u32 s_w[16];
    __shared__ u64 s_carry;
    const int lane = lane_id(), w = threadIdx.x >> 6;
    if (threadIdx.x == 0) s_carry = 0;
    __syncthreads();
    const u32 t_first = blk_tot ? blockIdx.x * PER * 1024u : 0u, t_end = blk_tot ? (t_first + PER * 1024u < T ? t_first + PER * 1024u : T) : T;
    for (u32 t0 = t_first; t0 < t_end; t0 += PER * 1024) {
        const u32 t = t0 + PER * threadIdx.x;
        u32 v[PER];
        if (t + PER <= T) {
#pragma unroll
            for (u32 q = 0; q < PER / 4; ++q) {
                const uint4 x = reinterpret_cast<const uint4*>(in + t)[q];
                v[4 * q] = x.x; v[4 * q + 1] = x.y; v[4 * q + 2] = x.z; v[4 * q + 3] = x.w;
                reinterpret_cast<uint4*>(in + t)[q] = make_uint4(0, 0, 0, 0);
            }
        } else {
#pragma unroll
            for (u32 k = 0; k < PER; ++k) { v[k] = t + k < T ? in[t + k] : 0; if (t + k < T) in[t + k] = 0; }
        }
        u32 sum = 0;
#pragma unroll
        for (u32 k = 0; k < PER; ++k) sum += v[k];
        const u32 inc = wave_incl_scan32(sum, lane);
        if (lane == WAVE - 1) s_w[w] = inc;
        __syncthreads();
        u64 off = s_carry;
        for (int i = 0; i < w; ++i) off += s_w[i];
        u64 e = off + inc - sum;
        if (t + PER <= T) {
#pragma unroll
            for (u32 q = 0; q < PER / 2; ++q) {
                reinterpret_cast<ulonglong2*>(out + t)[q] = make_ulonglong2(e, e + v[2 * q]);
                e += (u64)v[2 * q] + v[2 * q + 1];
            }
        } else {
#pragma unroll
            for (u32 k = 0; k < PER; ++k) { if (t + k < T) out[t + k] = e; e += v[k]; }
        }
        __syncthreads();
        if (threadIdx.x == 1023) s_carry = off + inc;
        __syncthreads();
    }
    if (blk_tot) { if (threadIdx.x == 0) blk_tot[blockIdx.x] = s_carry; return; }
    if (threadIdx.x == 0 && total_out) *total_out = s_carry;
    if (threadIdx.x == 0 && running) { const u64 r = *running; *base_out = r; *running = r + s_carry; }
}

template <u32 PER>
__global__ __launch_bounds__(1024) void scan_fix_kernel(u64* __restrict__ out, u32 T, const u64* __restrict__ blk_tot, u32 n_blk,
                                                        u64* __restrict__ total_out, u64* __restrict__ running, u64* __restrict__ base_out) {
    u64 off = 0, total = 0;
    for (u32 i = 0; i < n_blk; ++i) { const u64 v = blk_tot[i]; if (i < blockIdx.x) off += v; total += v; }
    if (blockIdx.x == 0 && threadIdx.x == 0) {
        if (total_out) *total_out = total;
        if (running) { const u64 r = *running; *base_out = r; *running = r + total; }
    }
    if (blockIdx.x == 0 || off == 0) return;
    const u32 t_first = blockIdx.x * PER * 1024u;
    for (u32 k = threadIdx.x; k < PER * 1024u && t_first + k < T; k += 1024) out[t_first + k] += off;
}

constexpr int K1_THREADS = FASTF_K1_THREADS, K1_IPT = FASTF_K1_IPT, K1_TILE = K1_THREADS * K1_IPT, K1_WAVES = K1_THREADS / WAVE;
static_assert(K1_THREADS == 512 && K1_IPT == 8, "K1a layout: 8 waves x 8 items x 64 lanes per tile");

constexpr u32 BLK_RECS = 256, BLK_GX = 0, BLK_UMI = 2048, BLK_META = 3072, BLK_CELL = 4096;
constexpr u32 NBLK_GX = 0, NBLK_UM = 1024, NBLK_CELL = 2048;
__host__ __device__ __forceinline__ u32 blk_cell_off(bool narrow) { return narrow ? NBLK_CELL : BLK_CELL; }
__host__ __device__ __forceinline__ u32 blk_run_bytes(bool c16, bool narrow = false) { return blk_cell_off(narrow) + (c16 ? 2u : 4u) * BLK_RECS; }
struct CellOut { void* p; u32 run; u32 off; };
__device__ __forceinline__ void put_cell(const CellOut o, bool c16, u64 idx, u32 v) {
    unsigned char* at = reinterpret_cast<unsigned char*>(o.p);
    u64 i = idx;
    if (o.run) { at += (idx / BLK_RECS) * o.run + o.off; i = idx % BLK_RECS; }
    if (c16) reinterpret_cast<unsigned short*>(at)[i] = (unsigned short)v; else reinterpret_cast<u32*>(at)[i] = v;
}
__device__ __forceinline__ u32 get_cell(const void* __restrict__ in, bool c16, u64 idx) {
    return c16 ? (u32)reinterpret_cast<const unsigned short*>(in)[idx] : reinterpret_cast<const u32*>(in)[idx];
}

__device__ __forceinline__ u32 get_cell_once(const void* __restrict__ in, bool c16, u64 idx) {
    return c16 ? (u32)ld_once<FASTF_NT_K1B != 0>(reinterpret_cast<const unsigned short*>(in) + idx)
               : ld_once<FASTF_NT_K1B != 0>(reinterpret_cast<const u32*>(in) + idx);
}

__device__ __forceinline__ u32 shard_of(u32 cell, u32 n_shards) {
    return (u32)((mix64((u64)cell) >> 32) % n_shards);
}

template <int AUX>
__global__ __launch_bounds__(K1_THREADS) void probe_cells_kernel(const u64* __restrict__ cb, u64 n, Table cells,
                                                                 const CellOut cell_out, bool c16, u32* __restrict__ tile_hits,
                                                                 u32* __restrict__ half_hits) {
    __shared__ u32 s_w[K1_WAVES];
    const int tid = threadIdx.x, lane = lane_id(), w = tid >> 6;
    const u64 base = (u64)blockIdx.x * K1_TILE + (u64)w * (K1_IPT * WAVE);
    u64 key[K1_IPT]; u32 cell[K1_IPT];
#pragma unroll
    for (int j = 0; j < K1_IPT; ++j) {
        const u64 idx = base + (u64)j * WAVE + lane;
        key[j] = idx < n ? cb[idx] : 0;
    }
    table_probe_batch<K1_IPT, AUX>(cells, key, cell);
    u32 hits = 0, hits_lo = 0;
#pragma unroll
    for (int j = 0; j < K1_IPT; ++j) {
        const u64 idx = base + (u64)j * WAVE + lane;
        if (idx < n) put_cell(cell_out, c16, idx, cell[j]);
        hits += (u32)__popcll(__ballot(cell[j] != 0));
        if (j == K1_IPT / 2 - 1) hits_lo = hits;
    }
    if (lane == 0) {
        s_w[w] = hits;
        half_hits[((u64)blockIdx.x * K1_WAVES + w) * 2] = hits_lo; half_hits[((u64)blockIdx.x * K1_WAVES + w) * 2 + 1] = hits - hits_lo;
    }
    __syncthreads();
    if (tid == 0) {
        u32 t = 0;
        for (int i = 0; i < K1_WAVES; ++i) t += s_w[i];
        tile_hits[blockIdx.x] = t;
    }
}

struct CellLds { const u32* image; u32 slot_bits; u32 bucket_mask; u32 family; u32 bytes; u32 seed; };
struct GeneLds { const u32* image; u32 words; u32 n_perm; u32 family; u64 vmin; u64 range; u32 bytes; u32 direct; };

__host__ __device__ __forceinline__ u32 cell_mix(u32 code, u32 seed) {
    u32 h = (code ^ seed) * 0x9E3779B1u; h ^= h >> 15; h *= 0x85EBCA77u; h ^= h >> 13;
    return h;
}


struct MissFilter { const u32* bits; u32 mask; };
__device__ __forceinline__ u32 filter_bit(u64 key) {
    const u32 h = (u32)key * 0x85EBCA77u + (u32)(key >> 32) * 0xC2B2AE3Du;
    return h ^ (h >> 13);
}

__global__ __launch_bounds__(K1_THREADS, 8) void probe_cells_filtered_kernel(const u64* __restrict__ cb, u64 n, Table cells, MissFilter f,
// ... 308 lines not shown
        }
        emit[j] = alive;
        if (p.n_shards == 1) {
            const u64 m = __ballot(alive);
            if (m) {
                u32 b = 0;
                if (lane == 0) b = atomicAdd(&s_shard_cnt[0], (u32)__popcll(m));
                b = __shfl(b, 0, WAVE);
                if (alive) pos[j] = b + rank_below(m);
            }
        } else if (alive) {
            pos[j] = atomicAdd(&s_shard_cnt[shard[j]], 1u);
        }
    }

    K1STAMP(4);
    n_hit = wave_sum32(n_hit); n_samp = wave_sum32(n_samp); n_valid = wave_sum32(n_valid);
    if (lane == 0) {
        if (n_hit) atomicAdd(&s_tot[0], (u64)n_hit);
        if (n_samp) atomicAdd(&s_tot[1], (u64)n_samp);
        if (n_valid) atomicAdd(&s_tot[2], (u64)n_valid);
    }
    if (errs) atomicOr(&s_err, errs);
    __syncthreads();
    if (tid >= 64 && tid < 64 + (int)p.n_shards) {
        const u32 s = tid - 64;
        const u32 c = s_shard_cnt[s];
        u64 b = c ? atomicAdd(&p.key_counts[s], (u64)c) : 0;
        if (b + c > p.shard_stride) { atomicOr(&p.counters[3], ERR_KEYS_FULL); b = ~0ULL; }
        s_shard_base[s] = b;
    }
    __syncthreads();
    K1STAMP(5);
#pragma unroll
    for (int j = 0; j < K1B_IPT; ++j) {
        if (emit[j]) {
            const u64 b = s_shard_base[shard[j]];
            if (b != ~0ULL) {
                if (p.vals) {
                    const u32 sub = p.wide_sub_bits ? wide_sub_of(umi[j], meta[j]) : 0u;
                    const u64 at = (u64)shard[j] * p.shard_stride + b + pos[j];
                    p.vals[at] = key[j];
                    p.keys[at] = ((((u64)cell[j] << p.wide_feat_bits) | feat[j]) << p.wide_sub_bits) | sub;
                } else p.keys[(u64)shard[j] * p.shard_stride + b + pos[j]] = key[j];
            }
        }
    }
    K1STAMP(6);
    };
    if (tid < 3) s_tot[tid] = 0;
    if (tid == 0) s_err = 0;
    if constexpr (LDS_GENES) {
        __syncthreads();
        for (u32 tile = blockIdx.x; tile < p.n_tiles; tile += gridDim.x) {
            do_tile(tile);
            __syncthreads();
        }
    } else {
        __syncthreads();
        do_tile(blockIdx.x);
        __syncthreads();
    }
    if (tid < 3 && s_tot[tid]) atomicAdd(&p.counters[tid], s_tot[tid]);
    if (tid == 3 && s_err) atomicOr(&p.counters[3], (u64)s_err);
}

constexpr int K1S_IPT = 4, K1S_UNIT = K1S_IPT * WAVE;
static_assert(K1_TILE % K1S_UNIT == 0 && K1_TILE / K1S_UNIT == 16, "16 units per K1a tile");
#ifndef FASTF_K1S_THREADS
#define FASTF_K1S_THREADS 768
#endif
constexpr int K1S_THREADS = FASTF_K1S_THREADS, K1S_THREADS_ROOMY = 1024;
static_assert(K1S_THREADS % (4 * WAVE) == 0 && K1S_THREADS <= 1024, "whole waves on every SIMD");

constexpr int K1S_SUB = 2, K1S_BINS = 256;
struct StreamParams {
    const u32* half_hits;
    u64 region_stride;
    u64* seg_count;
    u32* rgn_hist;
    u64* rgn_phys;
    u64 slot0;
    u32 hist_shift;
};

__device__ __forceinline__ u32 row16_sum_lane15(u32 x) {
    x += (u32)__builtin_amdgcn_update_dpp(0, (int)x, 0x111, 0xF, 0xF, true);
    x += (u32)__builtin_amdgcn_update_dpp(0, (int)x, 0x112, 0xF, 0xF, true);
    x += (u32)__builtin_amdgcn_update_dpp(0, (int)x, 0x114, 0xF, 0xF, true);
    x += (u32)__builtin_amdgcn_update_dpp(0, (int)x, 0x118, 0xF, 0xF, true);
    return (u32)__builtin_amdgcn_readlane((int)x, 15);
}

template <bool ROOMY, bool C16, bool DIRECT, bool BLOCKED = false, bool NARROW = false>
__global__ __launch_bounds__(ROOMY ? K1S_THREADS_ROOMY : K1S_THREADS, ROOMY ? 4 : 2 * K1S_THREADS / (4 * WAVE)) void filter_pack_stream_kernel(const PackParams p, const StreamParams sp) {
    static_assert(BLOCKED || !NARROW, "the narrow records exist as blocked runs only");
    constexpr int THREADS = ROOMY ? K1S_THREADS_ROOMY : K1S_THREADS, WAVES = THREADS / WAVE;
    __shared__ u64 s_tot[3];
    __shared__ u32 s_cursor[K1S_SUB], s_err;
    __shared__ u32 s_hist[K1S_SUB * K1S_BINS];
    extern __shared__ __attribute__((aligned(16))) unsigned char smem[];
    const int tid = threadIdx.x, lane = lane_id();
    const int w = __builtin_amdgcn_readfirstlane(tid >> 6);
    const u32* s_bitmap = reinterpret_cast<const u32*>(smem);
    const unsigned short* s_rank = reinterpret_cast<const unsigned short*>(smem + (size_t)p.genes.words * 4);
    const unsigned short* s_perm = s_rank + ((p.genes.words + 1u) & ~1u);
    const unsigned short* s_direct = reinterpret_cast<const unsigned short*>(smem);
    {
        const uint4* src = reinterpret_cast<const uint4*>(p.genes.image);
        uint4* dst = reinterpret_cast<uint4*>(smem);
        for (u32 i = tid; i < (p.genes.bytes + 15u) / 16u; i += THREADS) dst[i] = src[i];
    }
    if (tid < 3) s_tot[tid] = 0;
    if (tid < K1S_SUB) s_cursor[tid] = 0;
    if (tid == 0) s_err = 0;
    for (int i = tid; i < K1S_SUB * K1S_BINS; i += THREADS) s_hist[i] = 0;
    __syncthreads();

    constexpr bool NT = FASTF_NT_K1B != 0;
    u64* const region0 = p.keys + (u64)blockIdx.x * K1S_SUB * sp.region_stride;
    const bool hs_hi = sp.hist_shift >= 32u;
    const u64 draw_off = p.draw_base ? *p.draw_base : 0;
    u32 w_hit = 0, w_samp = 0, w_valid = 0, errs = 0;
    const u32 n_units = p.n_tiles * (u32)(K1_TILE / K1S_UNIT), ustep = gridDim.x * (u32)WAVES;
    const u32 n_live = (u32)((p.n + K1S_UNIT - 1) / K1S_UNIT);
    u32 u = blockIdx.x * (u32)WAVES + (u32)w;
    struct UnitRegs { u32 cell[K1S_IPT], umi[K1S_IPT], meta[NARROW ? 1 : K1S_IPT], dw, avail, sbit, nvalid; };
    UnitRegs ra, rb;
    using GxT = std::conditional_t<NARROW, u32, u64>;
    GxT gxk[K1S_IPT];
    u64 tb = 0; u32 hha = 0;
    u32 zlane = 0;
    asm volatile("" : "+v"(zlane));
    auto records_of = [&](const u32 uu) { return uu < n_live ? (u32)(p.n - (u64)uu * K1S_UNIT < (u64)K1S_UNIT ? p.n - (u64)uu * K1S_UNIT : (u64)K1S_UNIT) : 0u; };
    auto unit_run = [&](const u32 uu) { return BLOCKED ? p.blk + (u64)uu * blk_run_bytes(C16, NARROW) : nullptr; };
    auto meta_of = [&](const UnitRegs& r, const int j) -> u32 { if constexpr (NARROW) return r.umi[j]; else return r.meta[j]; };
    auto load_gx = [&](GxT (&g)[K1S_IPT], const u32 uu, const u32 nv) {
        const GxT* gx_u;
        if constexpr (BLOCKED) gx_u = reinterpret_cast<const GxT*>(unit_run(uu) + (NARROW ? NBLK_GX : BLK_GX));
        else gx_u = p.gx + (u64)uu * K1S_UNIT;
#pragma unroll
        for (int j = 0; j < K1S_IPT; ++j) {
            const u32 o = (u32)j * WAVE + (u32)lane;
            g[j] = ld_once<NT>(gx_u + (BLOCKED || o < nv ? o : nv - 1u));
        }
    };
    auto load_rest = [&](u32 (&c)[K1S_IPT], u32 (&um)[K1S_IPT], u32 (&me)[NARROW ? 1 : K1S_IPT], const u32 uu, const u32 nv) {
        const unsigned char* const run = unit_run(uu);
        const u64 base = (u64)uu * K1S_UNIT;
        const u32* const umi_u = BLOCKED ? reinterpret_cast<const u32*>(run + (NARROW ? NBLK_UM : BLK_UMI)) : p.umi + base;
        const u32* const meta_u = BLOCKED ? reinterpret_cast<const u32*>(run + BLK_META) : p.meta + base;
        const unsigned short* const c16_u = BLOCKED ? reinterpret_cast<const unsigned short*>(run + blk_cell_off(NARROW)) : reinterpret_cast<const unsigned short*>(p.cell) + base;
        const u32* const c32_u = BLOCKED ? reinterpret_cast<const u32*>(run + blk_cell_off(NARROW)) : reinterpret_cast<const u32*>(p.cell) + base;
#pragma unroll
        for (int j = 0; j < K1S_IPT; ++j) {
            const u32 o = (u32)j * WAVE + (u32)lane, oc = BLOCKED || o < nv ? o : nv - 1u;
            c[j] = C16 ? (u32)ld_once<NT>(c16_u + oc) : ld_once<NT>(c32_u + oc);
            um[j] = ld_once<NT>(umi_u + oc);
            if constexpr (!NARROW) me[j] = ld_once<NT>(meta_u + oc);
        }
    };
    struct Place { u32 avail, sbit; };
    auto place_unit = [&](u32& words, const u32 uu, const u64 tbv, const u32 hhu) {
        const u32 place = uu & 15u;
        const u64 rank0 = uniform64(tbv) + draw_off + row16_sum_lane15((u32)lane < place ? hhu : 0u);
        Place q;
// ... 62 lines not shown
            bool fam = true, in;
            u32 vi;
            if constexpr (NARROW) {
                const u32 v = (u32)k - 1u - (u32)p.genes.vmin;
                in = want & (v < (u32)p.genes.range);
                vi = in ? v : 0u;
            } else {
                fam = (u32)(k >> 44) == p.genes.family;
                const u64 v = (k & 0xFFFFFFFFFFFull) - p.genes.vmin;
                in = want & fam & (v < p.genes.range);
                vi = in ? (u32)v : 0u;
            }
            u32 f;
            if (DIRECT) f = s_direct[vi];
            else {
                const u32 wd = s_bitmap[vi >> 5], rk = s_rank[vi >> 5], bit = vi & 31u;
                const u32 pi = ((wd >> bit) & 1u) ? rk + __popc(wd & ((1u << bit) - 1u)) : 0u;
                f = ((wd >> bit) & 1u) ? s_perm[pi] : 0u;
            }
            f = in ? f : 0u;
            if constexpr (!NARROW) {
                if (__ballot(want & !fam)) { if (want & !fam) f = table_probe(p.feats, k); }
            }
            feat[j] = f;
        }
        __builtin_amdgcn_sched_barrier(0);
        load_gx(gxk, us, ns);
        __builtin_amdgcn_sched_barrier(0);
        u64 key[K1S_IPT], em[K1S_IPT];
        u32 n_keys = 0;
#pragma unroll
        for (int j = 0; j < K1S_IPT; ++j) {
            bool alive = (cell[j] != 0) & (keep[j] != 0);
            w_samp += (u32)__popcll(__ballot(alive));
            const u32 mj = meta_of(cur, j);
            alive = alive & (feat[j] != 0) & ((mj & META_HAS_UB) != 0);
            const bool ovf = NARROW ? umi_overflows_narrow(p.L, umi[j]) : umi_overflows_flat(p.L, umi[j], mj);
            if (__ballot(alive & ovf)) errs |= (u32)ERR_UMI_TOOLONG;
            key[j] = make_key_flat(p.L, cell[j], feat[j], umi[j], mj);
            em[j] = __ballot(alive);
            n_keys += (u32)__popcll(em[j]);
        }
        w_valid += n_keys;
        if (n_keys) {
            u32 pos0 = 0;
            if (lane == 0) pos0 = atomicAdd(&s_cursor[SUB], n_keys);
            pos0 = (u32)__builtin_amdgcn_readfirstlane((int)pos0);
            if ((u64)pos0 + n_keys > sp.region_stride) errs |= (u32)ERR_KEYS_FULL;
            else {
                u64* const region = region0 + (u64)SUB * sp.region_stride;
#pragma unroll
                for (int j = 0; j < K1S_IPT; ++j) {
                    if (__builtin_amdgcn_inverse_ballot_w64(em[j])) {
                        region[pos0 + rank_below(em[j])] = key[j];
                        const u32 dg = hs_hi ? (u32)(key[j] >> 32) >> (sp.hist_shift - 32u) : __builtin_amdgcn_alignbit((u32)(key[j] >> 32), (u32)key[j], sp.hist_shift);
                        (void)__hip_atomic_fetch_add(&s_hist[SUB * K1S_BINS + (dg & (K1S_BINS - 1))], 1u, __ATOMIC_RELAXED, __HIP_MEMORY_SCOPE_WORKGROUP);
                    }
                    pos0 += (u32)__popcll(em[j]);
                }
            }
        }
        u = un;
    };
    while (u < n_units) {
        one_unit(ra, rb, std::integral_constant<int, 0>{});
        if (u >= n_units) break;
        one_unit(rb, ra, std::integral_constant<int, 1>{});
    }
    if (lane == 0) {
        if (w_hit) atomicAdd(&s_tot[0], (u64)w_hit);
        if (w_samp) atomicAdd(&s_tot[1], (u64)w_samp);
        if (w_valid) atomicAdd(&s_tot[2], (u64)w_valid);
    }
    {
        u32 e = errs;
#pragma unroll
        for (int o = 32; o > 0; o >>= 1) e |= __shfl_xor(e, o, WAVE);
        if (lane == 0 && e) atomicOr(&s_err, e);
    }
    __syncthreads();
    const int te = w * WAVE + lane;
    if (te < 3 && s_tot[te]) atomicAdd(&p.counters[te], s_tot[te]);
    if (te == 3 && s_err) atomicOr(&p.counters[3], (u64)s_err);
    if (te >= 64 && te < 64 + K1S_SUB) {
        const u32 r = blockIdx.x * K1S_SUB + (u32)(te - 64);
        sp.seg_count[r] = s_cursor[te - 64];
        if (sp.rgn_hist) sp.rgn_phys[r] = sp.slot0 + (u64)r * sp.region_stride;
    }
    if (sp.rgn_hist)
        for (int i = te; i < K1S_SUB * K1S_BINS; i += THREADS) sp.rgn_hist[(u64)blockIdx.x * (K1S_SUB * K1S_BINS) + i] = s_hist[i];
}

template <bool NARROW>
__global__ __launch_bounds__(256) void block_records_kernel(const u64* __restrict__ gx, const u32* __restrict__ umi, const u32* __restrict__ meta,
                                                            u64 n, unsigned char* __restrict__ blk, u32 run, u32 family, const KeyLayout L) {
    const u64 units = (n + BLK_RECS - 1) / BLK_RECS, waves = (u64)gridDim.x * (blockDim.x / WAVE);
    const int lane = lane_id();
    for (u64 u = (u64)blockIdx.x * (blockDim.x / WAVE) + (threadIdx.x >> 6); u < units; u += waves) {
        unsigned char* const r = blk + u * run;
#pragma unroll
        for (int j = 0; j < (int)BLK_RECS / WAVE; ++j) {
            const u32 o = (u32)j * WAVE + (u32)lane;
            const u64 i = u * BLK_RECS + o;
            const bool in = i < n;
            if constexpr (NARROW) {
                const u64 k = in ? gx[i] : 0;
                const u32 um = in ? umi[i] : 0, me = in ? meta[i] : 0;
                const u64 v = k & 0xFFFFFFFFFFFull;
                reinterpret_cast<u32*>(r + NBLK_GX)[o] = ((k != 0) & ((u32)(k >> 44) == family) & (v < 0xFFFFFFFFull)) ? (u32)v + 1u : 0u;
                reinterpret_cast<u32*>(r + NBLK_UM)[o] = (um & ~0xFFu) | (me & 0xFFu) | (umi_overflows_flat(L, um, me) ? META_UMI_TOOLONG : 0u);
            } else {
                reinterpret_cast<u64*>(r + BLK_GX)[o] = in ? gx[i] : 0;
                reinterpret_cast<u32*>(r + BLK_UMI)[o] = in ? umi[i] : 0;
                reinterpret_cast<u32*>(r + BLK_META)[o] = in ? meta[i] : 0;
            }
        }
    }
}

constexpr int SP_THREADS = 256, SP_IPT = 8, SP_TILE = SP_THREADS * SP_IPT, MAX_SHARDS = 8;
__global__ __launch_bounds__(SP_THREADS) void shard_partition_kernel(const u64* __restrict__ seg_keys, const u64* __restrict__ seg_count,
                                                                     u64 region_stride, u32 cell_shift, u32 n_shards,
                                                                     u64* __restrict__ keys_out, u64 shard_stride,
                                                                     u64* __restrict__ key_counts, u64* __restrict__ err) {
    __shared__ u32 s_cnt[MAX_SHARDS];
    __shared__ u64 s_base[MAX_SHARDS];
    const int tid = threadIdx.x;
    const u64 cnt = seg_count[blockIdx.x];
    const u64* src = seg_keys + (u64)blockIdx.x * region_stride;
    for (u64 i0 = 0; i0 < cnt; i0 += SP_TILE) {
        if (tid < MAX_SHARDS) s_cnt[tid] = 0;
        __syncthreads();
        u64 key[SP_IPT]; u32 sh[SP_IPT], lp[SP_IPT];
#pragma unroll
        for (int j = 0; j < SP_IPT; ++j) {
            const u64 i = i0 + (u64)j * SP_THREADS + tid;
            key[j] = i < cnt ? src[i] : 0;
            sh[j] = 0; lp[j] = 0;
            if (i < cnt) { sh[j] = shard_of((u32)(key[j] >> cell_shift), n_shards); lp[j] = atomicAdd(&s_cnt[sh[j]], 1u); }
        }
        __syncthreads();
        if (tid < (int)n_shards) {
            const u32 c = s_cnt[tid];
            u64 bs = c ? atomicAdd(&key_counts[tid], (u64)c) : 0;
            if (bs + c > shard_stride) { atomicOr(err, ERR_KEYS_FULL); bs = ~0ull; }
            s_base[tid] = bs;
        }
        __syncthreads();
#pragma unroll
        for (int j = 0; j < SP_IPT; ++j) {
            const u64 i = i0 + (u64)j * SP_THREADS + tid;
            if (i < cnt && s_base[sh[j]] != ~0ull) keys_out[(u64)sh[j] * shard_stride + s_base[sh[j]] + lp[j]] = key[j];
        }
        __syncthreads();
    }
}

struct TileSeg { u64 delta1, hi1, delta2, hi2; };
struct SegMap { const u64* prefix; const TileSeg* tile_seg; u32 n_seg; u64 stride; };

__global__ __launch_bounds__(1024) void seg_scan_kernel(const u64* __restrict__ seg_count, u32 n_seg, u64* __restrict__ prefix,
                                                        u64* __restrict__ n_out, bool add = false) {
    __shared__ u64 s_w[16];
    __shared__ u64 s_carry;
    const int lane = lane_id(), w = threadIdx.x >> 6;
    if (threadIdx.x == 0) s_carry = 0;
    __syncthreads();
    for (u32 b0 = 0; b0 < n_seg; b0 += 1024) {
        const u32 b = b0 + threadIdx.x;
        const u64 v = b < n_seg ? seg_count[b] : 0;
        u64 inc = v;
#pragma unroll
        for (int o = 1; o < WAVE; o <<= 1) { const u64 x = __shfl_up(inc, o, WAVE); if (lane >= o) inc += x; }
        if (lane == WAVE - 1) s_w[w] = inc;
        __syncthreads();
        u64 off = s_carry;
        for (int i = 0; i < w; ++i) off += s_w[i];
        if (b < n_seg) prefix[b] = off + inc - v;
        __syncthreads();
        if (threadIdx.x == 1023) s_carry = off + inc;
        __syncthreads();
    }
    if (threadIdx.x == 0) { prefix[n_seg] = s_carry; *n_out = add ? *n_out + s_carry : s_carry; }
}

__device__ __forceinline__ u32 seg_region_of(const u64* __restrict__ prefix, u32 n_seg, u64 idx) {
    u32 lo = 0, hi = n_seg;
    while (hi - lo > 1) { const u32 mid = (lo + hi) >> 1; if (prefix[mid] <= idx) lo = mid; else hi = mid; }
    return lo;
}

__global__ __launch_bounds__(256) void seg_tiles_kernel(const u64* __restrict__ prefix, u32 n_seg, u64 stride, u32 tile_keys,
                                                        TileSeg* __restrict__ tile_seg) {
    const u64 total = prefix[n_seg];
    const u64 T = (total + tile_keys - 1) / tile_keys;
    for (u64 t = (u64)blockIdx.x * 256 + threadIdx.x; t < T; t += (u64)gridDim.x * 256) {
        const u64 first = t * tile_keys;
        const u32 b = seg_region_of(prefix, n_seg, first);
        TileSeg ts;
        ts.delta1 = (u64)b * stride - prefix[b]; ts.hi1 = prefix[b + 1];
        u32 b2 = b + 1;
        while (b2 < n_seg && prefix[b2 + 1] == ts.hi1) ++b2;
        if (b2 < n_seg) { ts.delta2 = (u64)b2 * stride - prefix[b2]; ts.hi2 = prefix[b2 + 1]; }
        else { ts.delta2 = 0; ts.hi2 = ts.hi1; }
        tile_seg[t] = ts;
    }
}

__device__ __forceinline__ u64 seg_phys(const SegMap m, u64 idx, const TileSeg ts) {
    if (idx < ts.hi1) return idx + ts.delta1;
    if (idx < ts.hi2) return idx + ts.delta2;
    const u32 b = seg_region_of(m.prefix, m.n_seg, idx);
    return (u64)b * m.stride + (idx - m.prefix[b]);
}

constexpr int RADIX = 256;
#ifndef FASTF_SORT_IPT_MAX
#define FASTF_SORT_IPT_MAX 8
#endif
#ifndef FASTF_SORT_THREADS
#define FASTF_SORT_THREADS 512
#endif
constexpr int SORT_THREADS = FASTF_SORT_THREADS, SORT_IPT = FASTF_SORT_IPT_MAX, SORT_TILE = SORT_THREADS * SORT_IPT, SORT_WAVES = SORT_THREADS / WAVE;

__device__ __forceinline__ u32 num_tiles(u64 n, u32 ipt) { const u64 t = (u64)ipt * SORT_THREADS; return (u32)((n + t - 1) / t); }
__device__ __forceinline__ u32 row_stride(u32 T) { return (T + 3u) & ~3u; }

__device__ __forceinline__ bool sort_streams(u64 n_keys) { return n_keys >= (24ull << 20); }

__device__ __forceinline__ u32 xcd_tile(u32 T, u32 r) {
    const u32 chunk = (T + 7u) >> 3;
    return r < chunk ? (blockIdx.x & 7u) * chunk + r : ~0u;
}

template <bool SEG>
__global__ __launch_bounds__(SORT_THREADS) void tile_count_kernel(const u64* __restrict__ keys, const u64* __restrict__ n_ptr,
                                                                  u32 shift, u32* __restrict__ cnt, u32 ipt, const SegMap seg) {
    __shared__ u32 s_h[4 * RADIX];
    const u64 n = *n_ptr;
    const u32 T = num_tiles(n, ipt);
    for (u32 r = blockIdx.x >> 3;; r += gridDim.x >> 3) {
        const u32 tile = xcd_tile(T, r);
        if (tile >= T) return;
        for (int i = threadIdx.x; i < 4 * RADIX; i += SORT_THREADS) s_h[i] = 0;
        __syncthreads();
        const u64 base = (u64)tile * ipt * SORT_THREADS;
        u32* my = s_h + (threadIdx.x & 3) * RADIX;
        u64 k[SORT_IPT];
        if constexpr (SEG) {
            const TileSeg ts = seg.tile_seg[tile];
#pragma unroll
            for (int j = 0; j < SORT_IPT; ++j) {
                const u64 idx = base + (u64)j * SORT_THREADS + threadIdx.x;
                k[j] = (j < (int)ipt && idx < n) ? ld_once<FASTF_NT_SORT != 0>(keys + seg_phys(seg, idx, ts)) : 0;
            }
        } else if (sort_streams(n)) {
#pragma unroll
            for (int j = 0; j < SORT_IPT; ++j) {
                const u64 idx = base + (u64)j * SORT_THREADS + threadIdx.x;
                k[j] = (j < (int)ipt && idx < n) ? ld_once<FASTF_NT_SORT != 0>(keys + idx) : 0;
            }
        } else {
#pragma unroll
            for (int j = 0; j < SORT_IPT; ++j) {
                const u64 idx = base + (u64)j * SORT_THREADS + threadIdx.x;
                k[j] = (j < (int)ipt && idx < n) ? keys[idx] : 0;
// ... 141 lines not shown
    __syncthreads();
    STAMP(2);

    u32 run = 0, inc = 0, ginc = 0;
    if (tid < RADIX) {
#pragma unroll
        for (int i = 0; i < SORT_WAVES; ++i) { const u32 c = s_whist[i * RADIX + tid]; s_whist[i * RADIX + tid] = run; run += c; }
        inc = wave_incl_scan32(run, lane);
        ginc = wave_incl_scan32(g_tot, lane);
        if (lane == WAVE - 1) { s_wtot[w] = inc; s_wtot[4 + w] = ginc; }
    }
    __syncthreads();
    if (tid < RADIX) {
        u32 o = 0, go = 0;
        for (int i = 0; i < w; ++i) { o += s_wtot[i]; go += s_wtot[4 + i]; }
        const u32 lstart = o + inc - run;
        s_start[tid] = lstart;
        s_delta[tid] = (go + ginc - g_tot) + g_off - lstart;
    }
    __syncthreads();
    STAMP(3);

#pragma unroll
    for (int j = 0; j < SORT_IPT; ++j) {
        if (j >= ipt) break;
        const u32 li = wbase + j * WAVE + lane;
        const u32 d = (FULL || li < n_valid) ? digit_of<SHIFT>(key[j], rshift) : 255u;
        const u32 p = s_start[d] + wh[d] + rnk[j];
        s_keys[p] = key[j];
        if constexpr (VALS) s_vals[p] = val[j];
    }
    __syncthreads();
    STAMP(4);

#pragma unroll
    for (int j = 0; j < SORT_IPT; ++j) {
        if (j >= ipt) break;
        const u32 pidx = j * SORT_THREADS + tid;
        if (FULL || pidx < n_valid) {
            const u64 k = s_keys[pidx];
            const u32 d = digit_of<SHIFT>(k, rshift);
            out[(u64)(u32)(s_delta[d] + pidx)] = k;
            if constexpr (VALS) vout[(u64)(u32)(s_delta[d] + pidx)] = s_vals[pidx];
        }
    }
    STAMP(5);
#ifdef FASTF_STAMPS
    __builtin_amdgcn_s_waitcnt(0);
    STAMP(6);
#endif
#undef STAMP
    return run;
}

template <int SHIFT, bool SEG = false, bool VALS = false>
__global__ __launch_bounds__(SORT_THREADS, VALS ? 4 : 8) void scatter_kernel(const u64* __restrict__ in, u64* __restrict__ out,
                                                               const u64* __restrict__ n_ptr,
                                                               const u32* __restrict__ off, const u32* __restrict__ bin_tot,
                                                               u32 ipt, u32 rshift, const SegMap seg, u64* stamps,
                                                               const u64* __restrict__ vin = nullptr, u64* __restrict__ vout = nullptr) {
    extern __shared__ __attribute__((aligned(16))) unsigned char smem[];
    const u64 n = *n_ptr;
    const u32 T = num_tiles(n, ipt);
    const u32 tile_keys = ipt * SORT_THREADS;
    const bool streams = sort_streams(n);
    for (u32 r = blockIdx.x >> 3;; r += gridDim.x >> 3) {
#ifdef FASTF_NO_XCD_SWIZZLE
        const u32 tile = (r << 3) | (blockIdx.x & 7u);
#else
        const u32 tile = xcd_tile(T, r);
#endif
        if (tile >= T) return;
        const u64 base = (u64)tile * tile_keys;
        const u32 n_valid = (u32)((n - base) < (u64)tile_keys ? (n - base) : (u64)tile_keys);
        int tid = (int)threadIdx.x;
        asm volatile("" : "+v"(tid));
        const u32 g_off = tid < RADIX ? off[(u64)tid * row_stride(T) + tile] : 0u;
        if (n_valid == tile_keys) (void)scatter_tile<SHIFT, true, SEG, VALS>(in, out, base, n_valid, tile, g_off, bin_tot, (int)ipt, smem, rshift, seg, tid, streams, stamps, vin, vout);
        else (void)scatter_tile<SHIFT, false, SEG, VALS>(in, out, base, n_valid, tile, g_off, bin_tot, (int)ipt, smem, rshift, seg, tid, streams, stamps, vin, vout);
        if constexpr (VALS) __syncthreads();
    }
}

constexpr u32 RGN_BLK = 64;
static_assert(K1S_BINS == RADIX, "K1b's region histograms are histograms of a sort digit");
__global__ __launch_bounds__(RADIX) void rgn_scan_blocks_kernel(u32* __restrict__ hist, u32 R, u32* __restrict__ blk_sum) {
    const u32 d = threadIdx.x, r0 = blockIdx.x * RGN_BLK, r1 = r0 + RGN_BLK < R ? r0 + RGN_BLK : R;
    u32 acc = 0;
    for (u32 r = r0; r < r1; r += 8) {
        u32 v[8];
#pragma unroll
        for (u32 k = 0; k < 8; ++k) v[k] = r + k < r1 ? hist[(u64)(r + k) * RADIX + d] : 0u;
#pragma unroll
        for (u32 k = 0; k < 8; ++k) { if (r + k < r1) hist[(u64)(r + k) * RADIX + d] = acc; acc += v[k]; }
    }
    blk_sum[(u64)blockIdx.x * RADIX + d] = acc;
}
__global__ __launch_bounds__(RADIX) void rgn_scan_fix_kernel(u32* __restrict__ hist, u32 R, const u32* __restrict__ blk_sum, u32 n_blk,
                                                             u32* __restrict__ bin_tot) {
    const u32 d = threadIdx.x, w = blockIdx.x;
    u32 off = 0, tot = 0;
    for (u32 i = 0; i < n_blk; ++i) { const u32 v = blk_sum[(u64)i * RADIX + d]; off += i < w ? v : 0u; tot += v; }
    if (w == 0) bin_tot[d] = tot;
    if (off == 0) return;
    const u32 r0 = w * RGN_BLK, r1 = r0 + RGN_BLK < R ? r0 + RGN_BLK : R;
    for (u32 r = r0; r < r1; ++r) hist[(u64)r * RADIX + d] += off;
}
__global__ __launch_bounds__(SORT_THREADS, 8) void scatter_regions_kernel(const u64* __restrict__ keys, u64* __restrict__ out,
                                                                           const u64* __restrict__ rgn_phys, const u64* __restrict__ rgn_count,
                                                                           const u32* __restrict__ hist_excl, const u32* __restrict__ bin_tot,
                                                                           u32 R, u32 ipt, u32 rshift, bool streams) {
    extern __shared__ __attribute__((aligned(16))) unsigned char smem[];
    const u32 tile_keys = ipt * SORT_THREADS;
    const SegMap none{nullptr, nullptr, 0, 0};
    for (u32 i = blockIdx.x >> 3;; i += gridDim.x >> 3) {
        const u32 r = xcd_tile(R, i);
        if (r >= R) return;
        const u64 cnt = rgn_count[r];
        const u64* const in = keys + rgn_phys[r];
        u32 acc = threadIdx.x < RADIX ? hist_excl[(u64)r * RADIX + threadIdx.x] : 0u;
        for (u64 base = 0; base < cnt; base += tile_keys) {
            const u32 n_valid = (u32)(cnt - base < (u64)tile_keys ? cnt - base : (u64)tile_keys);
            int tid = (int)threadIdx.x;
            asm volatile("" : "+v"(tid));
            u32 run;
            if (n_valid == tile_keys) run = scatter_tile<-1, true, false>(in, out, base, n_valid, r, acc, bin_tot, (int)ipt, smem, rshift, none, tid, streams);
            else run = scatter_tile<-1, false, false>(in, out, base, n_valid, r, acc, bin_tot, (int)ipt, smem, rshift, none, tid, streams);
            acc += run;
        }
    }
}
__global__ __launch_bounds__(256) void rgn_hist_kernel(const u64* __restrict__ keys, const u64* __restrict__ rgn_phys, const u64* __restrict__ rgn_count,
                                                       u32 R, u32 shift, u32* __restrict__ hist) {
    __shared__ u32 s_h[RADIX];
    for (u32 r = blockIdx.x; r < R; r += gridDim.x) {
        s_h[threadIdx.x] = 0;
        __syncthreads();
        const u64 cnt = rgn_count[r];
        const u64* const in = keys + rgn_phys[r];
        for (u64 i = threadIdx.x; i < cnt; i += 256) atomicAdd(&s_h[(u32)(in[i] >> shift) & 255u], 1u);
        __syncthreads();
        hist[(u64)r * RADIX + threadIdx.x] = s_h[threadIdx.x];
        __syncthreads();
    }
}


struct ReduceParams {
    const u64* keys; const u64* n_ptr;
    KeyLayout L; u32 feat_mask;
    u64* err;
    u32* feature; u32* cell; u32* count;
    u64* ukeys;
    u32* span_rows;
    u64* giant_list; u32* giant_n;
    u32 giant_max;
    const u64* vals; u32 wide_feat_bits;
};

constexpr u32 GIANT_MAX = 1u << 16, GIANT_PART = 1536, GIANT_LIST_CAP = 4096, GIANT_ITEM_WORDS = 4, GIANT_TAB = 4096;

#ifndef FASTF_K3_IPT
#define FASTF_K3_IPT 4
#endif
#ifndef FASTF_K3_THREADS
#define FASTF_K3_THREADS 512
#endif
constexpr int K3_THREADS = FASTF_K3_THREADS, K3_IPT = FASTF_K3_IPT, K3_TILE = K3_THREADS * K3_IPT, K3_WAVES = K3_THREADS / WAVE;
constexpr int K3_UNITS = K3_IPT * K3_WAVES;
static_assert(K3_UNITS <= WAVE, "one wave scans the (item, wave) units");

__host__ __device__ __forceinline__ u64 k3_chunk_start(u64 n, u32 b, u32 G) {
    const u64 T = (n + K3_TILE - 1) / K3_TILE;
    const u64 s = (T * b / G) * K3_TILE;
    return s < n ? s : n;
}

__device__ __forceinline__ u32 wave_min32(u32 v) {
#pragma unroll
    for (int o = 32; o > 0; o >>= 1) { const u32 t = (u32)__shfl_xor((int)v, o, WAVE); v = t < v ? t : v; }
    return v;
}
__device__ __forceinline__ u32 wave_max32(u32 v) {
#pragma unroll
    for (int o = 32; o > 0; o >>= 1) { const u32 t = (u32)__shfl_xor((int)v, o, WAVE); v = t > v ? t : v; }
    return v;
}

__device__ __forceinline__ void k3_barrier() { asm volatile("s_waitcnt lgkmcnt(0)\n\ts_barrier" ::: "memory"); }
// ... 614 lines not shown
```

fastf_amd/engine.py:

```python
import ctypes as C

import numpy as np

from . import _lib
from ._lib import Batch, Coo, EngineConfig, FastfError, ListsStruct, MT, UmiRows, check

HAS_CB, HAS_XF, HAS_GX, HAS_UB = 1, 2, 4, 8


def draw_threshold(rate_depth: float) -> int:
    return int(_lib.lib().fastf_draw_threshold(C.c_float(rate_depth)))


def mt_draws(seed: int, skip: int, n: int) -> np.ndarray:
    L = _lib.lib()
    mt = MT()
    L.fastf_mt_seed(C.byref(mt), seed)
    L.fastf_mt_skip(C.byref(mt), skip)
    out = np.empty(n, dtype=np.uint32)
    L.fastf_mt_fill(C.byref(mt), out.ctypes.data, n)
    return out


def sample_cells(n_cells: int, rate_cell: float, seed: int):
# ... 247 lines not shown

    def reseed(self, seed, skip=0):
        check(self._L.fastf_engine_reseed(self._h, seed, skip))

    def set_timing(self, on: bool):
        check(self._L.fastf_engine_set_timing(self._h, 1 if on else 0))

    def device_records(self, n_devices=1):
        out = (C.c_uint64 * max(1, n_devices))()
        check(self._L.fastf_engine_device_records(self._h, out, max(1, n_devices)))
        return [int(x) for x in out]

    def get_timing(self, which: int):
        ms, n = C.c_double(), C.c_uint64()
        check(self._L.fastf_engine_get_timing(self._h, which, C.byref(ms), C.byref(n)))
        return ms.value, n.value

    def reserve(self, max_records, max_keys):
        check(self._L.fastf_dev_reserve(self._h, max_records, max_keys))

    def dev_count_hits(self, d_cb, n, d_out, stream=0):
        check(self._L.fastf_dev_count_hits(self._h, d_cb, n, d_out, stream))

    def dev_count_hits_blocked(self, d_cb, n, d_blocked, d_out, stream=0):
        check(self._L.fastf_dev_count_hits_blocked(self._h, d_cb, n, d_blocked, d_out, stream))

    def block_bytes(self, n) -> int:
        v = C.c_uint64()
        check(self._L.fastf_dev_block_bytes(self._h, n, C.byref(v)))
        return int(v.value)

    def dev_block_records(self, d_gx, d_umi, d_meta, n, d_blocked, stream=0):
        check(self._L.fastf_dev_block_records(self._h, d_gx, d_umi, d_meta, n, d_blocked, stream))

    def dev_probe_pack(self, d_cb, d_gx, d_umi, d_meta, n, d_draws, n_draws, d_keys, shard_stride,
                       d_key_counts, d_counters, stream=0, d_draw_base=None, reuse_hits=False, segmented=False, blocked=False,
                       draw_bits=False):
        check(self._L.fastf_dev_probe_pack(self._h, d_cb, d_gx, d_umi, d_meta, n, d_draws, n_draws, d_draw_base,
                                           d_keys, shard_stride, d_key_counts, d_counters,
                                           (1 if reuse_hits else 0) | (2 if segmented else 0) | (8 if blocked else 0) | (16 if draw_bits else 0),
                                           stream))

    @property
    def wide(self) -> bool:
        return bool(self._L.fastf_engine_is_wide(self._h))

    def dev_probe_pack_wide(self, d_cb, d_gx, d_umi, d_meta, d_umi_ext, n, d_draws, n_draws, d_keys, d_vals, shard_stride,
                            d_key_counts, d_counters, stream=0, d_draw_base=None, reuse_hits=False, draw_bits=False):
        check(self._L.fastf_dev_probe_pack_wide(self._h, d_cb, d_gx, d_umi, d_meta, d_umi_ext or None, n, d_draws, n_draws, d_draw_base,
                                                d_keys, d_vals, shard_stride, d_key_counts, d_counters,
                                                (1 if reuse_hits else 0) | (16 if draw_bits else 0), stream))

    def dev_adopt_wide(self, d_keys, d_vals, n, stream=0):
        check(self._L.fastf_dev_adopt_wide(self._h, d_keys, d_vals, n, stream))

    def dev_draw_bits(self, d_draws, n_draws, d_bits_out, stream=0):
        check(self._L.fastf_dev_draw_bits(self._h, d_draws, n_draws, d_bits_out, stream))

    def dev_mt_decisions(self, seed, skip, n_draws, d_bits_out, stream=0):
        check(self._L.fastf_dev_mt_decisions(self._h, seed, skip, n_draws, d_bits_out, stream))

    def dev_mt_decisions_multi(self, seed, skip, n_draws, thresholds, d_planes_out, plane_stride_words, stream=0):
        t = np.ascontiguousarray(thresholds, dtype=np.uint64)
        check(self._L.fastf_dev_mt_decisions_multi(self._h, seed, skip, n_draws, t.ctypes.data, len(t), d_planes_out,
                                                   plane_stride_words, stream))

    def dev_cell_summary(self, d_cell, d_count, d_nnz, n_cells, d_umis_per_cell, d_genes_per_cell, stream=0):
        check(self._L.fastf_dev_cell_summary(self._h, d_cell, d_count, d_nnz, n_cells, d_umis_per_cell, d_genes_per_cell, stream))

    def dev_cell_hits(self, n, d_blocked, d_hits_per_cell, stream=0):
        check(self._L.fastf_dev_cell_hits(self._h, n, d_blocked or None, d_hits_per_cell, stream))

    def dev_cell_decisions(self, n, d_blocked, seed, skip, n_draws, d_thresholds, d_bits_out, stream=0):
        check(self._L.fastf_dev_cell_decisions(self._h, n, d_blocked or None, seed, skip, n_draws, d_thresholds, d_bits_out, stream))

    def probe_capacity(self, n) -> int:
        v = C.c_uint64()
        check(self._L.fastf_dev_probe_capacity(self._h, n, C.byref(v)))
        return int(v.value)

    def dev_set_regions(self, d_counts, n_regions, stride, d_n_out, stream=0):
        check(self._L.fastf_dev_set_regions(self._h, d_counts, n_regions, stride, d_n_out, stream))

    def dev_sort(self, d_keys, d_tmp, d_n, max_n, key_bits=None, stream=0, skip_low=False, segmented=False) -> bool:
        in_tmp = C.c_int(0)
        check(self._L.fastf_dev_sort(self._h, d_keys, d_tmp, d_n, max_n,
                                     self.key_bits if key_bits is None else key_bits,
                                     (2 if skip_low else 0) | (4 if segmented else 0), C.byref(in_tmp), stream))
        return bool(in_tmp.value)

    def dev_reduce(self, d_sorted, d_n, max_n, d_feature, d_cell, d_count, d_nnz, stream=0, skip_low=False, segmented=False):
        check(self._L.fastf_dev_reduce(self._h, d_sorted, d_n, max_n, d_feature, d_cell, d_count, d_nnz,
                                       (2 if skip_low else 0) | (8 if segmented else 0), stream))

    def dev_rows_gather(self, d_n, feature, cell, count, stream=0):
        check(self._L.fastf_dev_rows_gather(self._h, d_n, feature, cell, count, stream))

    @property
    def table_modes(self) -> str:
        c, g = C.c_int(), C.c_int()
        check(self._L.fastf_engine_table_modes(self._h, C.byref(c), C.byref(g)))
        return "cells:%s genes:%s" % ("LDS perfect hash" if c.value else "L2 open addressing",
                                      {0: "L2 open addressing", 1: "LDS bitmap+rank", 2: "LDS direct table"}[g.value])

    @property
    def cell_scratch_bytes(self) -> int:
        b = C.c_uint32()
        check(self._L.fastf_engine_cell_scratch_bytes(self._h, C.byref(b)))
        return b.value

    @property
    def skip_bits(self) -> int:
        b = C.c_uint32()
        check(self._L.fastf_engine_skip_bits(self._h, C.byref(b)))
        return b.value

    def sort_passes(self, skip_low=False) -> int:
        b = C.c_uint32()
        check(self._L.fastf_engine_sort_passes(self._h, 2 if skip_low else 0, C.byref(b)))
        return b.value

    def dev_umi_rows(self, d_sorted, d_n, max_n, d_ukeys, d_ncopy, d_nrows, stream=0):
        check(self._L.fastf_dev_umi_rows(self._h, d_sorted, d_n, max_n, d_ukeys, d_ncopy, d_nrows, stream))

    def dev_error_bits(self) -> int:
        b = C.c_uint64()
        check(self._L.fastf_dev_error_bits(self._h, C.byref(b)))
        return int(b.value)

    def dev_clear_error_bits(self, mask, stream=0):
        check(self._L.fastf_dev_clear_error_bits(self._h, mask, stream))

    def close(self):
        if getattr(self, "_h", None):
            self._L.fastf_engine_destroy(self._h)
            self._h = None

    def __del__(self):
        try:
            self.close()
        except Exception:
            pass


def _libc_free(ptr):
    libc = C.CDLL(None)
    libc.free.argtypes = [C.c_void_p]
    libc.free(ptr)
```

include/fastf_amd.h:

```cpp
#ifndef FASTF_AMD_H
#define FASTF_AMD_H

#include <stddef.h>
#include <stdint.h>

#ifdef __cplusplus
extern "C" {
#endif


extern int _umi_copies_flag;

int bam2db(char *bam_file, char *db_file, char *path_out, char *barcodes_file,
           char *features_file, float rate_cell, float rate_depth, unsigned int seed);

int cmd_bam2db(int argc, const char **argv);
void fastf_pick_devices(const char *devices, const char *device, int *dev0, int *dev_second);

#ifndef FASTF_NO_TREE_TYPES
#if !defined(FASTQ_FILTER_H)
typedef struct node { char *data; long int count; struct node *left; struct node *right; } node;
#endif
#if !defined(EXTRACT_H)
typedef struct CB_node { node *CR; char *CB; struct CB_node *left; struct CB_node *right; } CB_node;
// ... 97 lines not shown
    uint64_t        key_capacity;
    uint32_t        n_devices;
    const int32_t  *devices;
} fastf_engine_config_t;

typedef struct fastf_batch {
    const uint64_t *cb_key;
    const uint64_t *gx_key;
    const uint32_t *umi;
    const uint32_t *meta;
    size_t          n;
    const uint32_t *umi_ext;
} fastf_batch_t;

typedef struct fastf_coo {
    const uint32_t *feature;
    const uint32_t *cell;
    const uint32_t *count;
    size_t          nnz;
} fastf_coo_t;

typedef struct fastf_umi_rows {
    const uint32_t *feature, *cell, *n_copy;
    const uint32_t *umi;
    const uint8_t  *nonnull;
    size_t          n;
} fastf_umi_rows_t;

int fastf_sweep_cells_from_coo(const fastf_coo_t *coo, uint32_t n_cells, uint64_t *umis_per_cell, uint32_t *genes_per_cell, uint64_t *umis);
int fastf_sweep_summary_row(float rate_cell, float rate_depth, uint32_t seed, const uint64_t counters[3], uint64_t nnz, uint64_t umis,
                            const uint64_t *umis_per_cell, const uint32_t *genes_per_cell, uint32_t n_cells, char *buf, size_t cap);

int  fastf_engine_create(const fastf_engine_config_t *cfg, fastf_engine_t **out);
void fastf_engine_destroy(fastf_engine_t *e);
int  fastf_engine_push(fastf_engine_t *e, const fastf_batch_t *batch);
int  fastf_engine_push_draws(fastf_engine_t *e, const fastf_batch_t *batch,
                             const uint32_t *draws, size_t n_draws);
int  fastf_engine_push_pinned(fastf_engine_t *e, const fastf_batch_t *batch);
int  fastf_engine_wait_input(fastf_engine_t *e);
void *fastf_pinned_alloc(size_t bytes);
void  fastf_pinned_free(void *p);
int   fastf_pinned_register(void *p, size_t bytes);
void  fastf_pinned_unregister(void *p);
int   fastf_debug_live_registrations(void);
int  fastf_engine_finish(fastf_engine_t *e, fastf_coo_t *coo, uint64_t counters[3]);
int  fastf_engine_lend_rows(fastf_engine_t *e, void *pinned, size_t bytes);
int  fastf_engine_umi_rows(fastf_engine_t *e, fastf_umi_rows_t *rows);
int  fastf_engine_device_records(const fastf_engine_t *e, uint64_t *records, uint32_t n);
int  fastf_engine_reset(fastf_engine_t *e);
int  fastf_engine_key_bits(const fastf_engine_t *e, uint32_t *cell_bits, uint32_t *feature_bits,
                           uint32_t *umi_bits, uint32_t *total_bits);

typedef struct fastf_taghist fastf_taghist_t;
typedef struct fastf_taghist_result {
    uint64_t n_records;
    uint64_t n_valid;
    uint64_t n_key1_present;
    const uint64_t *key1, *count1, *first1; size_t n1;
    const uint32_t *pair_k1;
    const uint64_t *pair_key2, *pair_count, *pair_first; size_t n_pairs;
} fastf_taghist_result_t;
int  fastf_taghist_create(int device, fastf_taghist_t **out);
void fastf_taghist_destroy(fastf_taghist_t *h);
int  fastf_taghist_push(fastf_taghist_t *h, const uint64_t *key1, const uint64_t *key2, size_t n);
uint64_t *fastf_taghist_reserve_device(fastf_taghist_t *h, size_t n);
void *fastf_taghist_stream(fastf_taghist_t *h);
int  fastf_taghist_push_device(fastf_taghist_t *h, const uint64_t *d_key1, size_t n);
int  fastf_taghist_finish(fastf_taghist_t *h, fastf_taghist_result_t *result);


int fastf_dev_count_hits(fastf_engine_t *e, const uint64_t *d_cb_key, uint64_t n,
                         uint64_t *d_hits_out, void *stream);

int fastf_dev_probe_pack(fastf_engine_t *e,
                         const uint64_t *d_cb_key, const uint64_t *d_gx_key,
                         const uint32_t *d_umi, const uint32_t *d_meta, uint64_t n,
                         const uint32_t *d_draws, uint64_t n_draws, const uint64_t *d_draw_base,
                         uint64_t *d_keys_out, uint64_t shard_stride,
                         uint64_t *d_key_counts, uint64_t *d_counters, uint32_t flags, void *stream);
#define FASTF_PROBE_REUSE_HITS 1u
#define FASTF_PROBE_SEGMENTED 2u
int fastf_dev_probe_capacity(const fastf_engine_t *e, uint64_t n, uint64_t *key_slots);

int fastf_dev_block_bytes(const fastf_engine_t *e, uint64_t n, uint64_t *bytes);
int fastf_dev_block_records(fastf_engine_t *e, const uint64_t *d_gx_key, const uint32_t *d_umi, const uint32_t *d_meta,
                            uint64_t n, void *d_blocked, void *stream);
#define FASTF_PROBE_BLOCKED 8u
int fastf_dev_count_hits_blocked(fastf_engine_t *e, const uint64_t *d_cb_key, uint64_t n, void *d_blocked,
                                 uint64_t *d_hits_out, void *stream);
#define FASTF_PROBE_DRAW_BITS 16u
int fastf_dev_draw_bits(fastf_engine_t *e, const uint32_t *d_draws, uint64_t n_draws, uint32_t *d_bits_out, void *stream);
int fastf_dev_mt_decisions(fastf_engine_t *e, uint32_t seed, uint64_t skip, uint64_t n_draws, uint32_t *d_bits_out, void *stream);

int fastf_dev_mt_decisions_multi(fastf_engine_t *e, uint32_t seed, uint64_t skip, uint64_t n_draws, const uint64_t *thresholds,
                                 uint32_t n_thresholds, uint32_t *d_planes_out, uint64_t plane_stride_words, void *stream);
int fastf_dev_cell_summary(fastf_engine_t *e, const uint32_t *d_cell, const uint32_t *d_count, const uint64_t *d_nnz, uint32_t n_cells,
                           uint64_t *d_umis_per_cell, uint32_t *d_genes_per_cell, void *stream);

int fastf_dev_cell_hits(fastf_engine_t *e, uint64_t n, const void *d_blocked, uint32_t *d_hits_per_cell, void *stream);
int fastf_dev_cell_decisions(fastf_engine_t *e, uint64_t n, const void *d_blocked, uint32_t seed, uint64_t skip, uint64_t n_draws,
                             const uint64_t *d_thresholds, uint32_t *d_bits_out, void *stream);

int fastf_engine_is_wide(const fastf_engine_t *e);
int fastf_dev_probe_pack_wide(fastf_engine_t *e, const uint64_t *d_cb_key, const uint64_t *d_gx_key, const uint32_t *d_umi,
                              const uint32_t *d_meta, const uint32_t *d_umi_ext, uint64_t n,
                              const uint32_t *d_draws, uint64_t n_draws, const uint64_t *d_draw_base,
                              uint64_t *d_keys_out, uint64_t *d_vals_out, uint64_t shard_stride, uint64_t *d_key_counts,
                              uint64_t *d_counters, uint32_t flags, void *stream);
int fastf_dev_adopt_wide(fastf_engine_t *e, const uint64_t *d_keys, const uint64_t *d_vals, uint64_t n, void *stream);

#define FASTF_SORT_SKIP_LOW   2u
#define FASTF_SORT_SEGMENTED  4u
int fastf_dev_set_regions(fastf_engine_t *e, const uint64_t *d_counts, uint32_t n_regions, uint64_t stride,
                          uint64_t *d_n_out, void *stream);
int fastf_engine_skip_bits(const fastf_engine_t *e, uint32_t *bits);
int fastf_engine_sort_passes(const fastf_engine_t *e, uint32_t flags, uint32_t *passes);
int fastf_engine_table_modes(const fastf_engine_t *e, int *cells_in_lds, int *genes_in_lds);
int fastf_engine_cell_scratch_bytes(const fastf_engine_t *e, uint32_t *bytes);
int fastf_dev_sort(fastf_engine_t *e, uint64_t *d_keys, uint64_t *d_tmp,
                   const uint64_t *d_n, uint64_t max_n, uint32_t key_bits, uint32_t flags,
                   int *sorted_in_tmp, void *stream);

#define FASTF_REDUCE_SEGMENTED 8u
int fastf_dev_reduce(fastf_engine_t *e, const uint64_t *d_sorted, const uint64_t *d_n,
                     uint64_t max_n, uint32_t *d_feature, uint32_t *d_cell,
                     uint32_t *d_count, uint64_t *d_nnz, uint32_t flags, void *stream);
int fastf_dev_rows_gather(fastf_engine_t *e, const uint64_t *d_n, uint32_t *feature, uint32_t *cell,
                          uint32_t *count, void *stream);

int fastf_dev_umi_rows(fastf_engine_t *e, const uint64_t *d_sorted, const uint64_t *d_n,
                       uint64_t max_n, uint64_t *d_ukeys, uint32_t *d_ncopy,
                       uint64_t *d_nrows, void *stream);

int fastf_dev_reserve(fastf_engine_t *e, uint64_t max_records, uint64_t max_keys);

#define FASTF_ERR_RUN_TOO_LONG 16u
int fastf_dev_error_bits(fastf_engine_t *e, uint64_t *bits);
int fastf_dev_clear_error_bits(fastf_engine_t *e, uint64_t mask, void *stream);

const char *fastf_kernel_names(void);

#ifdef __cplusplus
}
#endif
#endif
```

Measured before the change: 107.8 billion.

## Fold key total into K1b atomics and replace two-kernel region scan with one

```diff
diff --git a/fastf_amd/_lib.py b/fastf_amd/_lib.py
--- a/fastf_amd/_lib.py
+++ b/fastf_amd/_lib.py
@@ -186,6 +186,10 @@
     L.fastf_dev_block_bytes.argtypes = [vp, u64, C.POINTER(u64)]
     L.fastf_dev_block_records.argtypes = [vp, vp, vp, vp, u64, vp, vp]
     L.fastf_dev_set_regions.argtypes = [vp, vp, u32, u64, vp, vp]
+    if hasattr(L, "fastf_dev_k1_geometry"):
+        L.fastf_dev_k1_geometry.argtypes = [vp, u64, C.POINTER(u32), C.POINTER(u32)]
+    if hasattr(L, "fastf_dev_set_regions_walk"):
+        L.fastf_dev_set_regions_walk.argtypes = [vp, vp, vp, u32, u64, vp, vp]
     if hasattr(L, "fastf_dev_draw_bits") or not os.environ.get("FASTF_LIB_OVERRIDE"):
         L.fastf_dev_draw_bits.argtypes = [vp, vp, u64, vp, vp]
     if hasattr(L, "fastf_dev_mt_decisions"):
diff --git a/fastf_amd/csrc/umi_engine.hip b/fastf_amd/csrc/umi_engine.hip
--- a/fastf_amd/csrc/umi_engine.hip
+++ b/fastf_amd/csrc/umi_engine.hip
@@ -229,8 +229,9 @@
     DevBuf d_segkeys;
     DevBuf d_segcount, d_segprefix, d_tileseg;
     u32 giant_parity = 0;
+    bool seg_prefix_stale = false;
     u32 seg_n = 0; u64 seg_stride = 0;
-    DevBuf d_rgn_phys, d_rgn_hist, d_rgn_blk;
+    DevBuf d_rgn_phys, d_rgn_hist;
     u32 rgn_hist_n = 0, rgn_hist_shift = 0;
     bool stream_mode = false, store_regions = false;
     bool narrow = false, genes_one_family = false;
@@ -606,7 +607,7 @@
     DevBuf* all[] = {&e->tab_cells, &e->tab_feats, &e->img_cells, &e->img_genes, &e->d_cell_filter, &e->d_keys, &e->d_tmp, &e->d_small, &e->d_feature, &e->d_cell,
                      &e->d_count, &e->d_ukeys, &e->d_ncopy, &e->d_cellidx, &e->d_tilecnt, &e->d_tilebase, &e->d_binbase, &e->d_cnt, &e->d_rg_feature, &e->d_rg_cell, &e->d_rg_count, &e->d_rg_ukeys, &e->d_spanrows, &e->d_spanbase, &e->d_giant, &e->d_scanblk,
                      &e->d_halfhits, &e->d_segcount, &e->d_segprefix, &e->d_tileseg, &e->d_segkeys, &e->d_vals, &e->d_vtmp,
-                     &e->d_rgn_phys, &e->d_rgn_hist, &e->d_rgn_blk};
+                     &e->d_rgn_phys, &e->d_rgn_hist};
     for (DevBuf* b : all) b->release();
     if (e->s_compute) (void)hipStreamDestroy(e->s_compute);
     if (e->s_copy) (void)hipStreamDestroy(e->s_copy);
@@ -723,20 +724,21 @@
 static u64* g_k1_stamps = nullptr;
 extern "C" void fastf_debug_set_k1_stamps(void* p) { g_k1_stamps = (u64*)p; }
 
-static void launch_scan_tiles(fastf_engine* e, int slot, hipStream_t s, u32* in, u64* out, u32 T, u64* total_out, u64* running, u64* base_out) {
+static void launch_scan_tiles(fastf_engine* e, int slot, hipStream_t s, u32* in, u64* out, u32 T, u64* total_out, u64* running, u64* base_out,
+                              u64* zero_out = nullptr) {
     constexpr u32 CHUNK = 16u * 1024u;
     const u32 n_blk = (T + CHUNK - 1) / CHUNK;
     if (n_blk <= 1 || n_blk > 64 || e->d_scanblk.ensure(2 * 64 * sizeof(u64))) {
-        hipLaunchKernelGGL(scan_tiles_kernel<16>, dim3(1), dim3(1024), 0, s, in, out, T, total_out, running, base_out, (u64*)nullptr);
+        hipLaunchKernelGGL(scan_tiles_kernel<16>, dim3(1), dim3(1024), 0, s, in, out, T, total_out, running, base_out, (u64*)nullptr, zero_out);
         return;
     }
     u64* const blk = (u64*)e->d_scanblk.p + 64 * slot;
-    hipLaunchKernelGGL(scan_tiles_kernel<16>, dim3(n_blk), dim3(1024), 0, s, in, out, T, (u64*)nullptr, (u64*)nullptr, (u64*)nullptr, blk);
-    hipLaunchKernelGGL(scan_fix_kernel<16>, dim3(n_blk), dim3(1024), 0, s, out, T, (const u64*)blk, n_blk, total_out, running, base_out);
+    hipLaunchKernelGGL(scan_tiles_kernel<16>, dim3(n_blk), dim3(1024), 0, s, in, out, T, (u64*)nullptr, (u64*)nullptr, (u64*)nullptr, blk, (u64*)nullptr);
+    hipLaunchKernelGGL(scan_fix_kernel<16>, dim3(n_blk), dim3(1024), 0, s, out, T, (const u64*)blk, n_blk, total_out, running, base_out, zero_out);
 }
 
 static int launch_probe_cells(fastf_engine* e, const u64* cb, u64 n, u64* d_total_out, hipStream_t s,
-                              u64* d_running = nullptr, u64* d_base_out = nullptr, void* blk = nullptr) {
+                              u64* d_running = nullptr, u64* d_base_out = nullptr, void* blk = nullptr, u64* d_zero_out = nullptr) {
     if (reserve_workspace(e, blk ? 0 : n, 0, n)) return 1;
     const u32 tiles = (u32)((n + K1_TILE - 1) / K1_TILE);
     const CellOut cout = blk ? CellOut{blk, blk_run_bytes(e->cell16, e->narrow), blk_cell_off(e->narrow)} : CellOut{e->d_cellidx.p, 0u, 0u};
@@ -759,7 +761,7 @@
     }
     t_end(e, s, &e->t_k1_ms, &e->t_k1_n);
     dbg_sync(s, "K1a probe_cells");
-    launch_scan_tiles(e, 0, s, (u32*)e->d_tilecnt.p, (u64*)e->d_tilebase.p, tiles, d_total_out, d_running, d_base_out);
+    launch_scan_tiles(e, 0, s, (u32*)e->d_tilecnt.p, (u64*)e->d_tilebase.p, tiles, d_total_out, d_running, d_base_out, d_zero_out);
     dbg_sync(s, "K1a tile scan");
     HIP_OK(hipGetLastError());
     return 0;
@@ -1086,7 +1088,9 @@
                         u64* wide_vals = nullptr, const u32* wide_ext = nullptr) {
     if (segmented && !app) { e->seg_n = 0; e->rgn_hist_n = 0; }
     if (n == 0) return 0;
-    if (!reuse_hits && launch_probe_cells(e, cb, n, nullptr, s, d_running, d_running ? const_cast<u64*>(draw_base) : nullptr, blk)) return 1;
+    const bool k1b_total = segmented && (app || !reuse_hits);
+    if (!reuse_hits && launch_probe_cells(e, cb, n, nullptr, s, d_running, d_running ? const_cast<u64*>(draw_base) : nullptr, blk,
+                                          k1b_total && !app ? key_counts : nullptr)) return 1;
     const u32 tiles = (u32)((n + K1_TILE - 1) / K1_TILE);
     PackParams p{};
     p.cell = e->d_cellidx.p; p.cell16 = e->cell16; p.gx = gx; p.umi = umi; p.meta = meta; p.n = n;
@@ -1128,7 +1132,7 @@
         if (e->d_segprefix.ensure(((size_t)n_rgn + 1) * sizeof(u64))) return 1;
         StreamParams sp{(const u32*)e->d_halfhits.p, region, (u64*)e->d_segcount.p + rgn0,
                         stream_shards ? nullptr : (u32*)e->d_rgn_hist.p + (size_t)rgn0 * RADIX, (u64*)e->d_rgn_phys.p + rgn0,
-                        app ? app->slot0 : 0ull, e->skip_bits};
+                        app ? app->slot0 : 0ull, e->skip_bits, k1b_total ? key_counts : nullptr};
         const int variant = (e->genes_blocks_per_cu >= 2 ? 0 : 4) | (e->cell16 ? 2 : 0) | (e->lds_genes.direct ? 1 : 0);
 #define FPS(R, C, D) do { if (blk && e->narrow) hipLaunchKernelGGL((filter_pack_stream_kernel<R, C, D, true, true>), dim3(grid), dim3(R ? K1S_THREADS_ROOMY : K1S_THREADS), e->lds_genes.bytes, s, p, sp); \
                           else if (blk) hipLaunchKernelGGL((filter_pack_stream_kernel<R, C, D, true>), dim3(grid), dim3(R ? K1S_THREADS_ROOMY : K1S_THREADS), e->lds_genes.bytes, s, p, sp); \
@@ -1143,10 +1147,9 @@
         if (stream_shards) {
             hipLaunchKernelGGL(shard_partition_kernel, dim3(n_rgn), dim3(SP_THREADS), 0, s, (const u64*)e->d_segkeys.p, (const u64*)e->d_segcount.p,
                                region, e->L.cell_shift, e->n_shards, keys, stride, key_counts, counters + 3);
-        } else if (app) {
-            hipLaunchKernelGGL(seg_scan_kernel, dim3(1), dim3(1024), 0, s, (const u64*)e->d_segcount.p + rgn0, n_rgn, (u64*)e->d_segprefix.p, key_counts, true);
-        } else {
-            hipLaunchKernelGGL(seg_scan_kernel, dim3(1), dim3(1024), 0, s, (const u64*)e->d_segcount.p, n_rgn, (u64*)e->d_segprefix.p, key_counts, false);
+        } else if (!app) {
+            if (!k1b_total) hipLaunchKernelGGL(seg_scan_kernel, dim3(1), dim3(1024), 0, s, (const u64*)e->d_segcount.p, n_rgn, (u64*)e->d_segprefix.p, key_counts, false);
+            e->seg_prefix_stale = k1b_total;
             e->seg_n = n_rgn; e->seg_stride = region;
             e->rgn_hist_n = n_rgn; e->rgn_hist_shift = e->skip_bits;
         }
@@ -1221,6 +1224,16 @@
     u32 grid; u64 region;
     stream_geometry(e, (n + K1_TILE - 1) / K1_TILE, &grid, &region);
     *key_slots = (u64)grid * K1S_SUB * region;
+    return 0;
+} FASTF_CATCH_INT
+
+extern "C" int fastf_dev_k1_geometry(const fastf_engine_t* e, uint64_t n, uint32_t* tile_records, uint32_t* k1a_grid) FASTF_TRY {
+    if (!e || !tile_records || !k1a_grid) return set_err("null argument");
+    if (e->multi) return set_err("fastf_dev_k1_geometry: device-level calls take a single-device engine");
+    const u32 tiles = (u32)((n + K1_TILE - 1) / K1_TILE);
+    *tile_records = (u32)K1_TILE;
+    *k1a_grid = e->use_lds_cells ? std::min<u32>(e->cells_blocks_per_cu * g_cu_count, (tiles + 1) / 2)
+              : e->cell_filter.bits ? std::min<u32>(tiles, 4 * g_cu_count) : tiles;
     return 0;
 } FASTF_CATCH_INT
 
@@ -1287,6 +1300,10 @@
         walk = e->rgn_hist_n == e->seg_n && e->rgn_hist_shift == low_bit && !no_walk && !vals;
         if (!walk) {
             if (!e->seg_stride) return set_err("internal error: regions without a common stride need their histograms");
+            if (e->seg_prefix_stale) {
+                hipLaunchKernelGGL(seg_scan_kernel, dim3(1), dim3(1024), 0, s, (const u64*)e->d_segcount.p, e->seg_n, (u64*)e->d_segprefix.p, (u64*)nullptr, false);
+                e->seg_prefix_stale = false;
+            }
             seg = SegMap{(const u64*)e->d_segprefix.p, (const TileSeg*)e->d_tileseg.p, e->seg_n, e->seg_stride};
             hipLaunchKernelGGL(seg_tiles_kernel, dim3(std::min<u32>((T + 255) / 256, 1024)), dim3(256), 0, s, seg.prefix, seg.n_seg,
                                seg.stride, ipt * SORT_THREADS, (TileSeg*)e->d_tileseg.p);
@@ -1298,10 +1315,8 @@
         u64* dst = (q & 1) ? keys : tmp;
         const u32 shift = low_bit + 8 * q;
         if (q == 0 && walk) {
-            const u32 R = e->seg_n, n_blk = (R + RGN_BLK - 1) / RGN_BLK;
-            if (e->d_rgn_blk.ensure((size_t)n_blk * RADIX * sizeof(u32))) return 1;
-            hipLaunchKernelGGL(rgn_scan_blocks_kernel, dim3(n_blk), dim3(RADIX), 0, s, (u32*)e->d_rgn_hist.p, R, (u32*)e->d_rgn_blk.p);
-            hipLaunchKernelGGL(rgn_scan_fix_kernel, dim3(n_blk), dim3(RADIX), 0, s, (u32*)e->d_rgn_hist.p, R, (const u32*)e->d_rgn_blk.p, n_blk, bintot);
+            const u32 R = e->seg_n;
+            hipLaunchKernelGGL(rgn_scan_kernel, dim3(RADIX), dim3(RGN_THREADS), 0, s, (u32*)e->d_rgn_hist.p, R, bintot);
             t_begin(e, s);
             hipLaunchKernelGGL(scatter_regions_kernel, dim3(tile_grid(R)), dim3(SORT_THREADS), scatter_smem_bytes(ipt), s, src, dst,
                                (const u64*)e->d_rgn_phys.p, (const u64*)e->d_segcount.p, (const u32*)e->d_rgn_hist.p, (const u32*)bintot, R, ipt, shift,
@@ -1335,7 +1350,27 @@
     if (e->d_segprefix.ensure(((size_t)n_regions + 1) * sizeof(u64))) return 1;
     hipLaunchKernelGGL(seg_scan_kernel, dim3(1), dim3(1024), 0, (hipStream_t)stream, (const u64*)d_counts, (u32)n_regions, (u64*)e->d_segprefix.p, (u64*)d_n_out);
     HIP_OK(hipGetLastError());
-    e->seg_n = n_regions; e->seg_stride = stride; e->rgn_hist_n = 0;
+    e->seg_n = n_regions; e->seg_stride = stride; e->rgn_hist_n = 0; e->seg_prefix_stale = false;
+    return 0;
+} FASTF_CATCH_INT
+
+extern "C" int fastf_dev_set_regions_walk(fastf_engine_t* e, const uint64_t* d_keys, const uint64_t* d_counts, uint32_t n_regions,
+                                          uint64_t stride, uint64_t* d_n_out, void* stream) FASTF_TRY {
+    if (!d_keys) return set_err("null argument");
+    if (fastf_dev_set_regions(e, d_counts, n_regions, stride, d_n_out, stream)) return 1;
+    NO_WIDE(e, "fastf_dev_set_regions_walk");
+    if (e->rgn_n) return set_err("fastf_dev_set_regions_walk on an engine that holds pushed chunks: fastf_engine_reset first");
+    if (grow_regions(e, n_regions)) return 1;
+    hipStream_t s = (hipStream_t)stream;
+    std::vector<u64> phys(n_regions);
+    for (u32 r = 0; r < n_regions; ++r) phys[r] = (u64)r * stride;
+    HIP_OK(hipMemcpyAsync(e->d_rgn_phys.p, phys.data(), (size_t)n_regions * sizeof(u64), hipMemcpyHostToDevice, s));
+    HIP_OK(hipMemcpyAsync(e->d_segcount.p, d_counts, (size_t)n_regions * sizeof(u64), hipMemcpyDeviceToDevice, s));
+    HIP_OK(hipStreamSynchronize(s));
+    hipLaunchKernelGGL(rgn_hist_kernel, dim3(std::min<u32>(n_regions, 8 * g_cu_count)), dim3(256), 0, s, (const u64*)d_keys, (const u64*)e->d_rgn_phys.p,
+                       (const u64*)e->d_segcount.p, (u32)n_regions, e->skip_bits, (u32*)e->d_rgn_hist.p);
+    HIP_OK(hipGetLastError());
+    e->rgn_hist_n = n_regions; e->rgn_hist_shift = e->skip_bits;
     return 0;
 } FASTF_CATCH_INT
 
diff --git a/fastf_amd/csrc/umi_kernels.hpp b/fastf_amd/csrc/umi_kernels.hpp
--- a/fastf_amd/csrc/umi_kernels.hpp
+++ b/fastf_amd/csrc/umi_kernels.hpp
@@ -404,7 +404,8 @@
 template <u32 PER>
 __global__ __launch_bounds__(1024) void scan_tiles_kernel(u32* __restrict__ in, u64* __restrict__ out, u32 T,
                                                           u64* __restrict__ total_out, u64* __restrict__ running = nullptr,
-                                                          u64* __restrict__ base_out = nullptr, u64* __restrict__ blk_tot = nullptr) {
+                                                          u64* __restrict__ base_out = nullptr, u64* __restrict__ blk_tot = nullptr,
+                                                          u64* __restrict__ zero_out = nullptr) {
     __shared__ u32 s_w[16];
     __shared__ u64 s_carry;
     const int lane = lane_id(), w = threadIdx.x >> 6;
@@ -451,16 +452,19 @@
     if (blk_tot) { if (threadIdx.x == 0) blk_tot[blockIdx.x] = s_carry; return; }
     if (threadIdx.x == 0 && total_out) *total_out = s_carry;
     if (threadIdx.x == 0 && running) { const u64 r = *running; *base_out = r; *running = r + s_carry; }
+    if (threadIdx.x == 0 && zero_out) *zero_out = 0;
 }
 
 template <u32 PER>
 __global__ __launch_bounds__(1024) void scan_fix_kernel(u64* __restrict__ out, u32 T, const u64* __restrict__ blk_tot, u32 n_blk,
-                                                        u64* __restrict__ total_out, u64* __restrict__ running, u64* __restrict__ base_out) {
+                                                        u64* __restrict__ total_out, u64* __restrict__ running, u64* __restrict__ base_out,
+                                                        u64* __restrict__ zero_out = nullptr) {
     u64 off = 0, total = 0;
     for (u32 i = 0; i < n_blk; ++i) { const u64 v = blk_tot[i]; if (i < blockIdx.x) off += v; total += v; }
     if (blockIdx.x == 0 && threadIdx.x == 0) {
         if (total_out) *total_out = total;
         if (running) { const u64 r = *running; *base_out = r; *running = r + total; }
+        if (zero_out) *zero_out = 0;
     }
     if (blockIdx.x == 0 || off == 0) return;
     const u32 t_first = blockIdx.x * PER * 1024u;
@@ -935,6 +939,7 @@
     u64* rgn_phys;
     u64 slot0;
     u32 hist_shift;
+    u64* key_total;
 };
 
 __device__ __forceinline__ u32 row16_sum_lane15(u32 x) {
@@ -1163,6 +1168,11 @@
     const int te = w * WAVE + lane;
     if (te < 3 && s_tot[te]) atomicAdd(&p.counters[te], s_tot[te]);
     if (te == 3 && s_err) atomicOr(&p.counters[3], (u64)s_err);
+    if (te == 4 && sp.key_total) {
+        u32 k = 0;
+        for (int i = 0; i < K1S_SUB; ++i) k += s_cursor[i];
+        if (k) atomicAdd(sp.key_total, (u64)k);
+    }
     if (te >= 64 && te < 64 + K1S_SUB) {
         const u32 r = blockIdx.x * K1S_SUB + (u32)(te - 64);
         sp.seg_count[r] = s_cursor[te - 64];
@@ -1262,7 +1272,7 @@
         if (threadIdx.x == 1023) s_carry = off + inc;
         __syncthreads();
     }
-    if (threadIdx.x == 0) { prefix[n_seg] = s_carry; *n_out = add ? *n_out + s_carry : s_carry; }
+    if (threadIdx.x == 0) { prefix[n_seg] = s_carry; if (n_out) *n_out = add ? *n_out + s_carry : s_carry; }
 }
 
 __device__ __forceinline__ u32 seg_region_of(const u64* __restrict__ prefix, u32 n_seg, u64 idx) {
@@ -1570,29 +1580,33 @@
     }
 }
 
-constexpr u32 RGN_BLK = 64;
 static_assert(K1S_BINS == RADIX, "K1b's region histograms are histograms of a sort digit");
-__global__ __launch_bounds__(RADIX) void rgn_scan_blocks_kernel(u32* __restrict__ hist, u32 R, u32* __restrict__ blk_sum) {
-    const u32 d = threadIdx.x, r0 = blockIdx.x * RGN_BLK, r1 = r0 + RGN_BLK < R ? r0 + RGN_BLK : R;
-    u32 acc = 0;
-    for (u32 r = r0; r < r1; r += 8) {
-        u32 v[8];
-#pragma unroll
-        for (u32 k = 0; k < 8; ++k) v[k] = r + k < r1 ? hist[(u64)(r + k) * RADIX + d] : 0u;
-#pragma unroll
-        for (u32 k = 0; k < 8; ++k) { if (r + k < r1) hist[(u64)(r + k) * RADIX + d] = acc; acc += v[k]; }
-    }
-    blk_sum[(u64)blockIdx.x * RADIX + d] = acc;
-}
-__global__ __launch_bounds__(RADIX) void rgn_scan_fix_kernel(u32* __restrict__ hist, u32 R, const u32* __restrict__ blk_sum, u32 n_blk,
-                                                             u32* __restrict__ bin_tot) {
-    const u32 d = threadIdx.x, w = blockIdx.x;
-    u32 off = 0, tot = 0;
-    for (u32 i = 0; i < n_blk; ++i) { const u32 v = blk_sum[(u64)i * RADIX + d]; off += i < w ? v : 0u; tot += v; }
-    if (w == 0) bin_tot[d] = tot;
-    if (off == 0) return;
-    const u32 r0 = w * RGN_BLK, r1 = r0 + RGN_BLK < R ? r0 + RGN_BLK : R;
-    for (u32 r = r0; r < r1; ++r) hist[(u64)r * RADIX + d] += off;
+constexpr u32 RGN_THREADS = 256, RGN_PER = 4, RGN_ROUND = RGN_THREADS * RGN_PER;
+__global__ __launch_bounds__(RGN_THREADS) void rgn_scan_kernel(u32* __restrict__ hist, u32 R, u32* __restrict__ bin_tot) {
+    __shared__ u32 s_w[RGN_THREADS / WAVE];
+    const u32 d = blockIdx.x, w = threadIdx.x >> 6;
+    const int lane = lane_id();
+    u32 carry = 0;
+    for (u32 r0 = 0; r0 < R; r0 += RGN_ROUND) {
+        const u32 r = r0 + RGN_PER * threadIdx.x;
+        u32 v[RGN_PER], sum = 0;
+#pragma unroll
+        for (u32 k = 0; k < RGN_PER; ++k) v[k] = r + k < R ? hist[(u64)(r + k) * RADIX + d] : 0u;
+#pragma unroll
+        for (u32 k = 0; k < RGN_PER; ++k) sum += v[k];
+        const u32 inc = wave_incl_scan32(sum, lane);
+        if (lane == WAVE - 1) s_w[w] = inc;
+        __syncthreads();
+        u32 off = carry, round = 0;
+#pragma unroll
+        for (u32 i = 0; i < RGN_THREADS / WAVE; ++i) { off += i < w ? s_w[i] : 0u; round += s_w[i]; }
+        u32 e = off + inc - sum;
+#pragma unroll
+        for (u32 k = 0; k < RGN_PER; ++k) { if (r + k < R) hist[(u64)(r + k) * RADIX + d] = e; e += v[k]; }
+        carry += round;
+        __syncthreads();
+    }
+    if (threadIdx.x == 0) bin_tot[d] = carry;
 }
 __global__ __launch_bounds__(SORT_THREADS, 8) void scatter_regions_kernel(const u64* __restrict__ keys, u64* __restrict__ out,
                                                                            const u64* __restrict__ rgn_phys, const u64* __restrict__ rgn_count,
diff --git a/fastf_amd/engine.py b/fastf_amd/engine.py
--- a/fastf_amd/engine.py
+++ b/fastf_amd/engine.py
@@ -353,6 +353,14 @@
     def dev_set_regions(self, d_counts, n_regions, stride, d_n_out, stream=0):
         check(self._L.fastf_dev_set_regions(self._h, d_counts, n_regions, stride, d_n_out, stream))
 
+    def k1_geometry(self, n):
+        t, g = C.c_uint32(0), C.c_uint32(0)
+        check(self._L.fastf_dev_k1_geometry(self._h, n, C.byref(t), C.byref(g)))
+        return t.value, g.value
+
+    def dev_set_regions_walk(self, d_keys, d_counts, n_regions, stride, d_n_out, stream=0):
+        check(self._L.fastf_dev_set_regions_walk(self._h, d_keys, d_counts, n_regions, stride, d_n_out, stream))
+
     def dev_sort(self, d_keys, d_tmp, d_n, max_n, key_bits=None, stream=0, skip_low=False, segmented=False) -> bool:
         in_tmp = C.c_int(0)
         check(self._L.fastf_dev_sort(self._h, d_keys, d_tmp, d_n, max_n,
diff --git a/include/fastf_amd.h b/include/fastf_amd.h
--- a/include/fastf_amd.h
+++ b/include/fastf_amd.h
@@ -203,6 +203,8 @@
 #define FASTF_PROBE_SEGMENTED 2u
 int fastf_dev_probe_capacity(const fastf_engine_t *e, uint64_t n, uint64_t *key_slots);
 
+int fastf_dev_k1_geometry(const fastf_engine_t *e, uint64_t n, uint32_t *tile_records, uint32_t *k1a_grid);
+
 int fastf_dev_block_bytes(const fastf_engine_t *e, uint64_t n, uint64_t *bytes);
 int fastf_dev_block_records(fastf_engine_t *e, const uint64_t *d_gx_key, const uint32_t *d_umi, const uint32_t *d_meta,
                             uint64_t n, void *d_blocked, void *stream);
@@ -234,6 +236,8 @@
 #define FASTF_SORT_SEGMENTED  4u
 int fastf_dev_set_regions(fastf_engine_t *e, const uint64_t *d_counts, uint32_t n_regions, uint64_t stride,
                           uint64_t *d_n_out, void *stream);
+int fastf_dev_set_regions_walk(fastf_engine_t *e, const uint64_t *d_keys, const uint64_t *d_counts, uint32_t n_regions,
+                               uint64_t stride, uint64_t *d_n_out, void *stream);
 int fastf_engine_skip_bits(const fastf_engine_t *e, uint32_t *bits);
 int fastf_engine_sort_passes(const fastf_engine_t *e, uint32_t flags, uint32_t *passes);
 int fastf_engine_table_modes(const fastf_engine_t *e, int *cells_in_lds, int *genes_in_lds);
```

Result: no change. 108.3 billion, median of 6 (+0.4%).
